# yeyupiaoling/MASR

Hardware: NVIDIA H100
Metric: audio_seconds_per_second (higher is better)
Workload: dtype f32 (GEMMs: fp16x2-split operands on wgmma, fp32 accumulate; fp32-grade results)

## Files before the change

include/masr_b200.h:

```cpp
#ifndef MASR_B200_H_
#define MASR_B200_H_

#include <stdint.h>

#ifdef __cplusplus
extern "C" {
#endif

#define MASR_ABI_VERSION 1

enum {
    MASR_OK = 0,
    MASR_ERR_INVALID_ARGUMENT = 10001,
    MASR_ERR_UNSUPPORTED_DEVICE = 10002,
    MASR_ERR_INTERNAL = 10003,
};

enum { MASR_STATUS_GAIN_EXCEEDED = 1 };

enum {
    MASR_EPI_BIAS = 0,
    MASR_EPI_BIAS_SILU = 1,
    MASR_EPI_BIAS_RELU = 2,
    MASR_EPI_BIAS_GLU = 3,
    MASR_EPI_BIAS_SCALE = 4,
    MASR_EPI_RESIDUAL = 5,
};

const char* masr_last_error(void);
int masr_abi_version(void);
int masr_check_device(void);


int masr_stage_waves_f32(const void* const* waves, const int64_t* lengths, int B, float* pinned, float* dev, int nthreads,
                         void* stream);

int masr_resample_f32(const float* x, const int64_t* x_offsets, const int* src_rates, int dst_rate, int B,
                      const double* table, int table_len, float* y, const int64_t* y_offsets, int64_t max_out,
                      int max_src_rate, void* stream);

int masr_fbank_workspace_bytes(int B, int64_t max_samples, int64_t* bytes_host);

int masr_wave_gain_f32(const float* wave, const int64_t* offsets, int B, int64_t max_samples, float target_db,
                       float max_gain_db, float* gain, int* status, void* workspace, void* stream);

int masr_fbank_f32(const float* wave, const int64_t* offsets, const float* gain, int B, int Fmax, float* feats,
                   int* num_frames, void* stream);


int masr_conv1_cmvn_relu_f32(const float* feats, const float* mean, const float* istd, const float* w1,
                             const float* b1, float* out, int B, int Fmax, int idim, int F1max, int W1, int C,
                             void* stream);

int masr_conv2_s2_relu_f32(const float* c1, const float* w2p, const float* b2, float* out, int B, int F1max,
                           int W1, int T2max, int W2, int C, void* stream);

int masr_gemm_f32(const float* A, int64_t lda, const float* W, const float* bias, const float* residual,
                  int64_t ldr, float* C, int64_t ldc, int M, int N, int K, int epilogue, float alpha,
                  void* stream);

int masr_gemm_tc_f16x2(const void* Ah, const void* Al, int64_t lda, const void* Wh, const void* Wl,
                       const float* bias, const float* residual, int64_t ldr, float* C, void* Ch, void* Cl,
                       int64_t ldc, int M, int N, int K, int epilogue, float alpha, void* stream);

int masr_ffn_tc_f16x2(const void* Ah, const void* Al, int64_t lda, const void* W1h, const void* W1l, const float* b1,
                      const void* W2h, const void* W2l, const float* b2, float* x, int64_t ldx, int M, int D, int F,
                      float alpha, void* stream);

int masr_gemm_tc_residual_ln_f16x2(const void* Ah, const void* Al, int64_t lda, const void* Wh, const void* Wl,
                                   const float* bias, const float* residual, int64_t ldr, float alpha, float* X,
                                   const float* gamma1, const float* beta1, const float* gamma2, const float* beta2,
                                   float* Y2, void* Yh, void* Yl, int64_t ldx, int M, int N, int K, float eps, void* stream);

int masr_gemm_tc_residual_postln_f16x2(const void* Ah, const void* Al, int64_t lda, const void* Wh, const void* Wl,
                                       const float* bias, const float* residual, int64_t ldr, float alpha, float* X,
                                       const float* gamma, const float* beta, const float* ada_scale, const float* ada_bias,
                                       void* Yh, void* Yl, int64_t ldx, int M, int N, int K, float eps, void* stream);

int masr_gemm_tc_lnpre_f16x2(const float* x, int64_t ldx, const float* gamma, const float* beta, float eps, void* Ah, void* Al,
                             int64_t lda, const void* Wh, const void* Wl, const float* bias, float* C, void* Ch, void* Cl,
                             int64_t ldc, int M, int N, int K, int epilogue, float alpha, void* stream);

int masr_ctc_head_argmax_tc_f16x2(const void* Ah, const void* Al, int64_t lda, const void* Wh, const void* Wl,
                                  const float* bias, int M, int V, int K, void* workspace, int64_t workspace_bytes,
                                  int* ids, float* maxp, void* stream);

int masr_conv1_cmvn_relu_planes_f16(const float* feats, const float* mean, const float* istd, const float* w1,
                                    const float* b1, void* planes_h, void* planes_l, int B, int Fmax, int idim,
                                    int F1max, int W1, int C, void* stream);
int masr_conv2_tc_f16x2(const void* c1h, const void* c1l, const void* Wh, const void* Wl, const float* bias,
                        float* out, void* outh, void* outl, int B, int F1, int T2, int C, void* stream);

int masr_split_f16(const float* x, void* h, void* l, int64_t n, void* stream);

int masr_layernorm_f32(const float* x, int64_t ldx, const float* gamma, const float* beta, float* y, int64_t ldy,
                       int M, int D, float eps, void* stream);

int masr_layernorm_split_f16(const float* x, int64_t ldx, const float* gamma, const float* beta, void* yh, void* yl,
                             int64_t ldy, int M, int D, float eps, void* stream);

int masr_layernorm2_split_f16(const float* x, int64_t ldx, const float* gamma1, const float* beta1, float* y1,
                              const float* gamma2, const float* beta2, float* y2, void* yh, void* yl, int64_t ldy, int M,
                              int D, float eps, void* stream);

int masr_layernorm_ada_split_f16(const float* x, int64_t ldx, const float* gamma, const float* beta, float* y,
                                 const float* ada_scale, const float* ada_bias, void* yh, void* yl, int64_t ldy, int M, int D,
                                 float eps, void* stream);
int masr_affine_split_f16(const float* x, const float* scale, const float* bias, void* yh, void* yl, int64_t M, int D,
                          void* stream);
int masr_dwconv_bn_silu_f32(const float* g, int64_t ldg, int64_t g_bstride, const float* w, const float* bias,
                            const float* bn_scale, const float* bn_shift, const float* pad_vec, float* y, void* yh, void* yl,
                            int64_t ldy, int64_t y_bstride, const int* in_lens, int B, int C, int kernel_size, int lpad,
                            int out_rows, void* stream);
int masr_time_reduce_dw_split_f16(const float* x, int64_t in_bstride, const float* w, const float* bias, void* yh, void* yl,
                                  int64_t out_bstride, const int* lens, int B, int out_rows, int k, int pad, int D,
                                  void* stream);
int masr_upsample2_add_f32(const float* saved, const float* z, float* out, int64_t full_bstride, int64_t half_bstride, int B,
                           int rows, int D, void* stream);

int masr_relpos_attention_f32(const float* Q, int64_t ldq, int64_t q_bstride, const float* K, const float* V,
                              int64_t ldk, int64_t k_bstride, const float* P, int64_t ldp, const float* pos_u,
                              const float* pos_v, float* O, void* Oh, void* Ol, int64_t ldo, int64_t o_bstride,
                              const int* q_lens, const int* k_lens, int B, int H, int d_k, int max_q, void* stream);

int masr_relpos_attention_tc(const float* Q, int64_t ldq, int64_t q_bstride, const void* Kh, const void* Kl, const void* Vh,
                             const void* Vl, int64_t ldk, int64_t k_bstride, const void* Ph, const void* Pl, int64_t ldp,
                             const float* pos_u, const float* pos_v, float* O, void* Oh, void* Ol, int64_t ldo,
                             int64_t o_bstride, const int* q_lens, const int* k_lens, int B, int H, int d_k, int max_q,
                             void* stream);

int masr_relpos_attention_tc5(const float* Q, int64_t ldq, int64_t q_bstride, const void* Kh, const void* Kl, const void* Vh,
                              const void* Vl, int64_t ldk, int64_t k_bstride, const void* Ph, const void* Pl, int64_t ldp,
                              int64_t table_rows, const float* pos_u, const float* pos_v, float* O, void* Oh, void* Ol,
                              int64_t ldo, int64_t o_bstride, const int* q_lens, const int* k_lens, int B, int H, int d_k,
                              int max_q, void* stream);

int masr_dwconv_ln_silu_f32(const float* g, int64_t ldg, int64_t g_bstride, const float* w, const float* bias,
                            const float* ln_gamma, const float* ln_beta, const float* pad_vec, float* y, void* yh,
                            void* yl, int64_t ldy, int64_t y_bstride, const int* in_lens, int B, int C,
                            int kernel_size, int lpad, int out_rows, float eps, void* stream);

int masr_dwconv_ln_silu_strided_f32(const float* g, int64_t ldg, int64_t g_bstride, const float* w, const float* bias,
                                    const float* ln_gamma, const float* ln_beta, const float* pad_vec, float* y, void* yh,
                                    void* yl, int64_t ldy, int64_t y_bstride, const int* in_lens, int B, int C,
                                    int kernel_size, int lpad, int stride, int out_rows, float eps, void* stream);

int masr_grouped_attention_f32(const float* Q, const float* K, const float* V, const float* P, int64_t ld, int64_t bstride,
                               const float* pos_u, const float* pos_v, float* O, void* Oh, void* Ol, const int* lens,
                               int B, int H, int d_k, int group, int max_t, void* stream);

int masr_grouped_attention_cache_f32(const float* Q, int64_t ldq, int64_t q_bstride, const float* K, const float* V,
                                     int64_t ldk, int64_t k_bstride, const float* P, const float* pos_u, const float* pos_v,
                                     float* O, void* Oh, void* Ol, const int* q_lens, const int* k_lens, int B, int H,
                                     int d_k, int group, int max_q, void* stream);

int masr_avgpool2_time_f32(const float* x, int64_t in_bstride, float* y, int64_t out_bstride, const int* lens, int B,
                           int out_rows, int D, void* stream);

int masr_lstm_step_f32(const float* gates_x, int64_t ldg, int64_t bstride, const float* Whh, const float* h_in_T,
                       float* h_out_T, float* c_state, float* out, void* outh, void* outl, int64_t ld_out, int col_off,
                       const int* lens, int B, int H, int step, int reverse, void* stream);

int masr_lstm_seq_workspace_bytes(int B, int H, int64_t* bytes);
int masr_lstm_seq_f32(const float* gates_x, int64_t ldg, int64_t bstride, const float* Whh, const float* h0_T, float* hN_T,
                      float* c_state, float* out, void* outh, void* outl, int64_t ld_out, int col_off, const int* lens, int B,
                      int H, int T, int reverse, void* workspace, int64_t workspace_bytes, void* stream);


int masr_stream_append_rows(const void* src0, const void* src1, int64_t src_pitch_bytes, int64_t col0_bytes, int row_bytes,
                            void* dst0, void* dst1, int64_t dst_pitch_bytes, int64_t cap, const int* base, const int* cnt,
                            int rows_per_slot, int S, void* stream);

int masr_stream_shift_cache(void* x0, void* x1, int64_t rows_per_slot, int lorder, int row_bytes, const int* cnt, int S,
                            void* stream);


int masr_ctc_frame_argmax_f32(const float* logits, int64_t ldl, int M, int V, int* ids, float* maxp, float* probs,
                              int64_t ldp, void* stream);

int masr_ctc_greedy_collapse(const int* ids, const float* maxp, int64_t bstride, const int* lens, int B, int blank,
                             int* tokens, int64_t tok_stride, int* ntok, float* psum, int* pcount, void* stream);

int masr_ctc_topk_f32(const float* logits, int64_t ldl, int M, int V, int top_n, float cutoff_prob, int* cand_id,
                      float* cand_logp, int* cand_cnt, void* stream);
int masr_ctc_prefix_beam_workspace(int B, int Tmax, int64_t* pool_floats_host, int64_t* trie_ints_per_utt_host);
int masr_ctc_prefix_beam(const int* cand_id, const float* cand_logp, const int* cand_cnt, int64_t bstride, const int* lens,
                         int B, int beam_size, int blank, float* pool, int* trie_parent, int* trie_tok, int64_t trie_cap,
                         int* out_tok, int64_t tok_stride, int* out_n, float* out_score, void* stream);

int masr_ctc_prefix_beam_state_size(int64_t* ints_per_utt, int64_t* floats_per_utt);
int masr_ctc_prefix_beam_stream(const int* cand_id, const float* cand_logp, const int* cand_cnt, int64_t bstride,
                                const int* lens, int B, int beam_size, int blank, float* pool, int* trie_parent,
                                int* trie_tok, int64_t trie_cap, int* state_i, float* state_f, int resume, int* out_tok,
                                int64_t tok_stride, int* out_n, float* out_score, void* stream);

typedef struct masr_lm_tables {
    const uint32_t* keys;
    const float* vals;
    const int* tok2lm;
    int order;
    int bos, eos;
    int vocab;
    int64_t off[8];
    int64_t mask[8];
} masr_lm_tables;

enum {
    MASR_LM_INFO_ORDER = 0, MASR_LM_INFO_CHAR_BASED = 1, MASR_LM_INFO_DICT_SIZE = 2, MASR_LM_INFO_VOCAB = 3,
    MASR_LM_INFO_KEY_WORDS = 4, MASR_LM_INFO_VAL_FLOATS = 5, MASR_LM_INFO_BOS = 6, MASR_LM_INFO_EOS = 7,
    MASR_LM_INFO_READ = 8,
    MASR_LM_INFO_KEPT = 14,
    MASR_LM_INFO_SLOTS = 20,
    MASR_LM_INFO_TABLE_BYTES = 26,
};

int masr_lm_load_arpa(const char* path_host, const char* vocab_host, int V, void** handle_host);
int masr_lm_info(const void* handle_host, int64_t* info_host);
int masr_lm_export(const void* handle_host, uint32_t* keys_host, float* vals_host, int* tok2lm_host,
                   masr_lm_tables* layout_host);
int masr_lm_free(void* handle_host);

int masr_lm_score_f32(const masr_lm_tables* lm_host, const int* ctx, const int* word, int Q, float* out, void* stream);

int masr_ctc_topk_blank_f32(const float* logits, int64_t ldl, int M, int V, int top_n, float cutoff_prob, int blank,
                            int* cand_id, float* cand_logp, int* cand_cnt, float* blank_logp, void* stream);

int masr_ctc_prefix_beam_lm(const int* cand_id, const float* cand_logp, const int* cand_cnt, const float* blank_logp,
                            int64_t bstride, const int* lens, int B, int beam_size, int blank, const masr_lm_tables* lm_host,
                            float alpha, float beta, float* pool, int* trie_parent, int* trie_tok, int64_t trie_cap,
                            int* out_tok, int64_t tok_stride, int* out_n, float* out_score, float* out_approx, void* stream);
int masr_ctc_prefix_beam_lm_state_size(int64_t* ints_per_utt, int64_t* floats_per_utt);
int masr_ctc_prefix_beam_lm_stream(const int* cand_id, const float* cand_logp, const int* cand_cnt, const float* blank_logp,
                                   int64_t bstride, const int* lens, int B, int beam_size, int blank,
                                   const masr_lm_tables* lm_host, float alpha, float beta, float* pool, int* trie_parent,
                                   int* trie_tok, int64_t trie_cap, int* state_i, float* state_f, int resume, int* out_tok,
                                   int64_t tok_stride, int* out_n, float* out_score, float* out_approx, void* stream);

int masr_ctc_prefix_beam_pool(const int* cand_id, const float* cand_logp, const int* cand_cnt, int64_t bstride,
                              const int* lens, int B, int beam_size, int blank, float* pool, int* trie_parent,
                              int* trie_tok, int64_t trie_cap, int* state_i, float* state_f, int* fresh, int* out_tok,
                              int64_t tok_stride, int* out_n, float* out_score, void* stream);
int masr_ctc_prefix_beam_lm_pool(const int* cand_id, const float* cand_logp, const int* cand_cnt, const float* blank_logp,
                                 int64_t bstride, const int* lens, int B, int beam_size, int blank,
                                 const masr_lm_tables* lm_host, float alpha, float beta, float* pool, int* trie_parent,
                                 int* trie_tok, int64_t trie_cap, int* state_i, float* state_f, int* fresh, int* out_tok,
                                 int64_t tok_stride, int* out_n, float* out_score, float* out_approx, void* stream);

#ifdef __cplusplus
}
#endif
#endif
```

masr_b200/_lib.py:

```python
from __future__ import annotations

import ctypes as C
import os
from typing import Optional

_HERE = os.path.dirname(os.path.abspath(__file__))
LIB_PATH = os.path.join(_HERE, "libmasr_b200.so")

OK = 0
EPI_BIAS, EPI_BIAS_SILU, EPI_BIAS_RELU, EPI_BIAS_GLU, EPI_BIAS_SCALE, EPI_RESIDUAL = range(6)
STATUS_GAIN_EXCEEDED = 1

_vp, _i, _i64, _f = C.c_void_p, C.c_int, C.c_int64, C.c_float


class LmTables(C.Structure):
    _fields_ = [("keys", _vp), ("vals", _vp), ("tok2lm", _vp), ("order", _i), ("bos", _i), ("eos", _i), ("vocab", _i),
                ("off", _i64 * 8), ("mask", _i64 * 8)]


_lmp = C.POINTER(LmTables)
LM_INFO_ORDER, LM_INFO_CHAR_BASED, LM_INFO_DICT_SIZE, LM_INFO_VOCAB, LM_INFO_KEY_WORDS, LM_INFO_VAL_FLOATS = range(6)
LM_INFO_READ, LM_INFO_KEPT, LM_INFO_SLOTS, LM_INFO_TABLE_BYTES = 8, 14, 20, 26

SIGNATURES = {
    "masr_abi_version": [],
    "masr_check_device": [],
    "masr_stage_waves_f32": [_vp, _vp, _i, _vp, _vp, _i, _vp],
    "masr_resample_f32": [_vp, _vp, _vp, _i, _i, _vp, _i, _vp, _vp, _i64, _i, _vp],
    "masr_fbank_workspace_bytes": [_i, _i64, C.POINTER(_i64)],
    "masr_wave_gain_f32": [_vp, _vp, _i, _i64, _f, _f, _vp, _vp, _vp, _vp],
    "masr_fbank_f32": [_vp, _vp, _vp, _i, _i, _vp, _vp, _vp],
    "masr_conv1_cmvn_relu_f32": [_vp, _vp, _vp, _vp, _vp, _vp, _i, _i, _i, _i, _i, _i, _vp],
    "masr_conv2_s2_relu_f32": [_vp, _vp, _vp, _vp, _i, _i, _i, _i, _i, _i, _vp],
    "masr_gemm_f32": [_vp, _i64, _vp, _vp, _vp, _i64, _vp, _i64, _i, _i, _i, _i, _f, _vp],
    "masr_gemm_tc_f16x2": [_vp, _vp, _i64, _vp, _vp, _vp, _vp, _i64, _vp, _vp, _vp, _i64, _i, _i, _i, _i, _f, _vp],
    "masr_ffn_tc_f16x2": [_vp, _vp, _i64, _vp, _vp, _vp, _vp, _vp, _vp, _vp, _i64, _i, _i, _i, _f, _vp],
    "masr_gemm_tc_residual_ln_f16x2": [_vp, _vp, _i64, _vp, _vp, _vp, _vp, _i64, _f, _vp, _vp, _vp, _vp, _vp, _vp, _vp, _vp, _i64,
                                       _i, _i, _i, _f, _vp],
    "masr_gemm_tc_residual_postln_f16x2": [_vp, _vp, _i64, _vp, _vp, _vp, _vp, _i64, _f, _vp, _vp, _vp, _vp, _vp, _vp, _vp, _i64,
                                           _i, _i, _i, _f, _vp],
    "masr_gemm_tc_lnpre_f16x2": [_vp, _i64, _vp, _vp, _f, _vp, _vp, _i64, _vp, _vp, _vp, _vp, _vp, _vp, _i64, _i, _i, _i, _i, _f,
                                 _vp],
    "masr_ctc_head_argmax_tc_f16x2": [_vp, _vp, _i64, _vp, _vp, _vp, _i, _i, _i, _vp, _i64, _vp, _vp, _vp],
    "masr_split_f16": [_vp, _vp, _vp, _i64, _vp],
    "masr_conv1_cmvn_relu_planes_f16": [_vp, _vp, _vp, _vp, _vp, _vp, _vp, _i, _i, _i, _i, _i, _i, _vp],
    "masr_conv2_tc_f16x2": [_vp, _vp, _vp, _vp, _vp, _vp, _vp, _vp, _i, _i, _i, _i, _vp],
    "masr_layernorm_f32": [_vp, _i64, _vp, _vp, _vp, _i64, _i, _i, _f, _vp],
    "masr_layernorm_split_f16": [_vp, _i64, _vp, _vp, _vp, _vp, _i64, _i, _i, _f, _vp],
    "masr_layernorm2_split_f16": [_vp, _i64, _vp, _vp, _vp, _vp, _vp, _vp, _vp, _vp, _i64, _i, _i, _f, _vp],
    "masr_layernorm_ada_split_f16": [_vp, _i64, _vp, _vp, _vp, _vp, _vp, _vp, _vp, _i64, _i, _i, _f, _vp],
    "masr_affine_split_f16": [_vp, _vp, _vp, _vp, _vp, _i64, _i, _vp],
    "masr_dwconv_bn_silu_f32": [_vp, _i64, _i64, _vp, _vp, _vp, _vp, _vp, _vp, _vp, _vp, _i64, _i64, _vp, _i, _i, _i, _i, _i, _vp],
    "masr_time_reduce_dw_split_f16": [_vp, _i64, _vp, _vp, _vp, _vp, _i64, _vp, _i, _i, _i, _i, _i, _vp],
    "masr_upsample2_add_f32": [_vp, _vp, _vp, _i64, _i64, _i, _i, _i, _vp],
    "masr_relpos_attention_f32": [_vp, _i64, _i64, _vp, _vp, _i64, _i64, _vp, _i64, _vp, _vp, _vp, _vp, _vp, _i64, _i64,
                                  _vp, _vp, _i, _i, _i, _i, _vp],
    "masr_relpos_attention_tc": [_vp, _i64, _i64, _vp, _vp, _vp, _vp, _i64, _i64, _vp, _vp, _i64, _vp, _vp, _vp, _vp, _vp, _i64,
                                 _i64, _vp, _vp, _i, _i, _i, _i, _vp],
    "masr_relpos_attention_tc5": [_vp, _i64, _i64, _vp, _vp, _vp, _vp, _i64, _i64, _vp, _vp, _i64, _i64, _vp, _vp, _vp, _vp, _vp,
                                  _i64, _i64, _vp, _vp, _i, _i, _i, _i, _vp],
    "masr_dwconv_ln_silu_f32": [_vp, _i64, _i64, _vp, _vp, _vp, _vp, _vp, _vp, _vp, _vp, _i64, _i64, _vp, _i, _i, _i, _i,
                                _i, _f, _vp],
    "masr_dwconv_ln_silu_strided_f32": [_vp, _i64, _i64, _vp, _vp, _vp, _vp, _vp, _vp, _vp, _vp, _i64, _i64, _vp, _i, _i, _i,
                                        _i, _i, _i, _f, _vp],
    "masr_grouped_attention_f32": [_vp, _vp, _vp, _vp, _i64, _i64, _vp, _vp, _vp, _vp, _vp, _vp, _i, _i, _i, _i, _i, _vp],
    "masr_grouped_attention_cache_f32": [_vp, _i64, _i64, _vp, _vp, _i64, _i64, _vp, _vp, _vp, _vp, _vp, _vp, _vp, _vp, _i, _i, _i,
                                         _i, _i, _vp],
    "masr_avgpool2_time_f32": [_vp, _i64, _vp, _i64, _vp, _i, _i, _i, _vp],
    "masr_lstm_step_f32": [_vp, _i64, _i64, _vp, _vp, _vp, _vp, _vp, _vp, _vp, _i64, _i, _vp, _i, _i, _i, _i, _vp],
    "masr_lstm_seq_workspace_bytes": [_i, _i, C.POINTER(_i64)],
    "masr_lstm_seq_f32": [_vp, _i64, _i64, _vp, _vp, _vp, _vp, _vp, _vp, _vp, _i64, _i, _vp, _i, _i, _i, _i, _vp, _i64, _vp],
    "masr_stream_append_rows": [_vp, _vp, _i64, _i64, _i, _vp, _vp, _i64, _i64, _vp, _vp, _i, _i, _vp],
    "masr_stream_shift_cache": [_vp, _vp, _i64, _i, _i, _vp, _i, _vp],
    "masr_ctc_frame_argmax_f32": [_vp, _i64, _i, _i, _vp, _vp, _vp, _i64, _vp],
    "masr_ctc_topk_f32": [_vp, _i64, _i, _i, _i, _f, _vp, _vp, _vp, _vp],
    "masr_ctc_prefix_beam_workspace": [_i, _i, C.POINTER(_i64), C.POINTER(_i64)],
    "masr_ctc_prefix_beam": [_vp, _vp, _vp, _i64, _vp, _i, _i, _i, _vp, _vp, _vp, _i64, _vp, _i64, _vp, _vp, _vp],
    "masr_ctc_prefix_beam_state_size": [C.POINTER(_i64), C.POINTER(_i64)],
    "masr_ctc_prefix_beam_stream": [_vp, _vp, _vp, _i64, _vp, _i, _i, _i, _vp, _vp, _vp, _i64, _vp, _vp, _i, _vp, _i64, _vp, _vp, _vp],
    "masr_ctc_greedy_collapse": [_vp, _vp, _i64, _vp, _i, _i, _vp, _i64, _vp, _vp, _vp, _vp],
    "masr_lm_load_arpa": [_vp, _vp, _i, C.POINTER(_vp)],
    "masr_lm_info": [_vp, C.POINTER(_i64)],
    "masr_lm_export": [_vp, _vp, _vp, _vp, _lmp],
    "masr_lm_free": [_vp],
    "masr_lm_score_f32": [_lmp, _vp, _vp, _i, _vp, _vp],
    "masr_ctc_topk_blank_f32": [_vp, _i64, _i, _i, _i, _f, _i, _vp, _vp, _vp, _vp, _vp],
    "masr_ctc_prefix_beam_lm": [_vp, _vp, _vp, _vp, _i64, _vp, _i, _i, _i, _lmp, _f, _f, _vp, _vp, _vp, _i64, _vp, _i64, _vp, _vp,
                                _vp, _vp],
    "masr_ctc_prefix_beam_lm_state_size": [C.POINTER(_i64), C.POINTER(_i64)],
    "masr_ctc_prefix_beam_lm_stream": [_vp, _vp, _vp, _vp, _i64, _vp, _i, _i, _i, _lmp, _f, _f, _vp, _vp, _vp, _i64, _vp, _vp, _i,
                                       _vp, _i64, _vp, _vp, _vp, _vp],
    "masr_ctc_prefix_beam_pool": [_vp, _vp, _vp, _i64, _vp, _i, _i, _i, _vp, _vp, _vp, _i64, _vp, _vp, _vp, _vp, _i64, _vp, _vp,
                                  _vp],
    "masr_ctc_prefix_beam_lm_pool": [_vp, _vp, _vp, _vp, _i64, _vp, _i, _i, _i, _lmp, _f, _f, _vp, _vp, _vp, _i64, _vp, _vp, _vp,
                                     _vp, _i64, _vp, _vp, _vp, _vp],
}


class MasrB200Error(RuntimeError):
    pass


_lib: Optional[C.CDLL] = None


def load() -> C.CDLL:
    global _lib
    if _lib is not None:
        return _lib
    if not os.path.exists(LIB_PATH):
        raise MasrB200Error(
            f"{LIB_PATH} not found: build it with `python -c 'import __graft_entry__ as g; g.build()'` "
            "(nvcc, sm_90a). masr_b200 has no CPU or PyTorch fallback.")
    lib = C.CDLL(LIB_PATH)
    lib.masr_last_error.restype = C.c_char_p
    lib.masr_last_error.argtypes = []
    for name, argtypes in SIGNATURES.items():
        fn = getattr(lib, name)
        fn.argtypes = argtypes
        fn.restype = C.c_int
    _lib = lib
    return lib


def last_error() -> str:
    return load().masr_last_error().decode("utf-8", "replace")


def check(rc: int, what: str):
    if rc != OK:
        raise MasrB200Error(f"{what} failed (code {rc}): {last_error()}")


def call(name: str, *args):
    check(getattr(load(), name)(*args), name)
```

masr_b200/csrc/ffn_tc.cu:

```cuda
#include <cuda.h>
#include <cuda_fp16.h>
#include <string.h>

#include "tc_common.cuh"

namespace masr {

namespace {

constexpr int FM = 64;
constexpr int FD = 256;
constexpr int FHC = 128;
constexpr int FBK = 32;
constexpr int F_STAGES = 4;
constexpr int F_STAGE_BYTES = 32768;
constexpr int F_H_BYTES = FM * FHC * 2 * 2;
constexpr int F_SUM_BYTES = FM * FD * 4;
constexpr int F_THREADS = 384;
constexpr int F_PRODUCER_REGS = 40, F_CONSUMER_REGS = 232;
constexpr uint32_t F_TX_A = 2 * FM * FBK * 2 + 2 * FHC * FBK * 2;
constexpr uint32_t F_TX_B = 2 * FD * FBK * 2;
constexpr size_t kFfnSmem = F_STAGES * F_STAGE_BYTES + F_H_BYTES + F_SUM_BYTES + 1024 + 256;
static_assert(kFfnSmem <= 232448, "ffn_tc shared memory exceeds the 227 KB per-CTA limit of sm_90");
static_assert(F_PRODUCER_REGS * 128 + F_CONSUMER_REGS * 256 <= 65536, "register file of the SM");

struct FfnMaps {
    CUtensorMap xh, xl;
    CUtensorMap w1h, w1l;
    CUtensorMap w2h, w2l;
};

struct FfnParams {
    const float* b1;
    const float* b2;
    float* x;
    int64_t ldx;
    int M, F;
    float alpha;
};

__device__ __forceinline__ void wgmma_m64n64k16_ss(float (&d)[32], uint64_t da, uint64_t db, uint32_t scale_d) {
    asm volatile(
        "{\n\t"
        ".reg .pred p;\n\t"
        "setp.ne.b32 p, %34, 0;\n\t"
        "wgmma.mma_async.sync.aligned.m64n64k16.f32.f16.f16 "
        "{%0, %1, %2, %3, %4, %5, %6, %7, %8, %9, %10, %11, %12, %13, %14, %15, "
        "%16, %17, %18, %19, %20, %21, %22, %23, %24, %25, %26, %27, %28, %29, %30, %31}, %32, %33, p, 1, 1, 0, 0;\n\t"
        "}"
        : "+f"(d[0]), "+f"(d[1]), "+f"(d[2]), "+f"(d[3]), "+f"(d[4]), "+f"(d[5]), "+f"(d[6]), "+f"(d[7]), "+f"(d[8]),
          "+f"(d[9]), "+f"(d[10]), "+f"(d[11]), "+f"(d[12]), "+f"(d[13]), "+f"(d[14]), "+f"(d[15]), "+f"(d[16]),
          "+f"(d[17]), "+f"(d[18]), "+f"(d[19]), "+f"(d[20]), "+f"(d[21]), "+f"(d[22]), "+f"(d[23]), "+f"(d[24]),
          "+f"(d[25]), "+f"(d[26]), "+f"(d[27]), "+f"(d[28]), "+f"(d[29]), "+f"(d[30]), "+f"(d[31])
        : "l"(da), "l"(db), "r"(scale_d));
}

__device__ __forceinline__ void bar_consumers() { asm volatile("bar.sync 1, 256;" ::: "memory"); }

__global__ void __launch_bounds__(F_THREADS, 1) ffn_tc_kernel(const __grid_constant__ FfnMaps maps, FfnParams p) {
    extern __shared__ uint8_t smem_raw[];
    uint8_t* smem = reinterpret_cast<uint8_t*>((reinterpret_cast<uintptr_t>(smem_raw) + 1023) & ~uintptr_t(1023));
    uint8_t* hbuf = smem + F_STAGES * F_STAGE_BYTES;
    uint8_t* sum = hbuf + F_H_BYTES;
    uint64_t* full_bar = reinterpret_cast<uint64_t*>(sum + F_SUM_BYTES);
    uint64_t* empty_bar = full_bar + F_STAGES;

    const int warp = threadIdx.x >> 5, lane = threadIdx.x & 31;
    const int nrb = (p.M + FM - 1) / FM;
    const int nch = p.F / FHC;

    if (warp == 8 && lane == 0) {
        tma_prefetch_desc(&maps.xh); tma_prefetch_desc(&maps.xl); tma_prefetch_desc(&maps.w1h);
        tma_prefetch_desc(&maps.w1l); tma_prefetch_desc(&maps.w2h); tma_prefetch_desc(&maps.w2l);
        for (int s = 0; s < F_STAGES; ++s) { mbar_init(&full_bar[s], 1); mbar_init(&empty_bar[s], 8); }
        asm volatile("fence.mbarrier_init.release.cluster;" ::: "memory");
    }
    __syncthreads();
    pdl_wait();
    pdl_launch_dependents();

    if (warp >= 8) {
        setmaxnreg_dec<F_PRODUCER_REGS>();
        if (warp == 8 && elect_one_sync()) {
            uint32_t kg = 0;
            auto acquire = [&](uint32_t tx) {
                const uint32_t s = kg % F_STAGES;
                mbar_wait(&empty_bar[s], ((kg / F_STAGES) & 1) ^ 1);
                mbar_expect_tx(&full_bar[s], tx);
                ++kg;
                return s;
            };
            for (int rb = blockIdx.x; rb < nrb; rb += gridDim.x) {
                const int m0 = rb * FM;
                for (int j = -1; j < nch; ++j) {
                    if (j >= 0) {
#pragma unroll 1
                        for (int kb = 0; kb < FHC / FBK; ++kb) {
                            const uint32_t s = acquire(F_TX_B);
                            uint8_t* st = smem + s * F_STAGE_BYTES;
                            tma_load_2d(&maps.w2h, &full_bar[s], st, j * FHC + kb * FBK, 0);
                            tma_load_2d(&maps.w2l, &full_bar[s], st + F_STAGE_BYTES / 2, j * FHC + kb * FBK, 0);
                        }
                    }
                    if (j + 1 < nch) {
#pragma unroll 1
                        for (int kb = 0; kb < FD / FBK; ++kb) {
                            const uint32_t s = acquire(F_TX_A);
                            uint8_t* st = smem + s * F_STAGE_BYTES;
                            tma_load_2d(&maps.xh, &full_bar[s], st, kb * FBK, m0);
                            tma_load_2d(&maps.xl, &full_bar[s], st + 4096, kb * FBK, m0);
                            tma_load_2d(&maps.w1h, &full_bar[s], st + 8192, kb * FBK, (j + 1) * FHC);
                            tma_load_2d(&maps.w1l, &full_bar[s], st + 16384, kb * FBK, (j + 1) * FHC);
                        }
                    }
                }
            }
        }
        __syncwarp();
    } else {
        setmaxnreg_inc<F_CONSUMER_REGS>();
        const int wg = warp >> 2, wi = warp & 3, q = lane & 3;
        const int tid = threadIdx.x & 127;
        const uint32_t h_base = smem_u32(hbuf);
        const uint32_t sum_base = smem_u32(sum) + wg * (F_SUM_BYTES / 2) + tid * 8;
        const uint32_t is_lane0 = lane == 0;
        auto release = [&](uint32_t s) {
            asm volatile("{\n\t.reg .pred p;\n\tsetp.ne.u32 p, %1, 0;\n\t@p mbarrier.arrive.shared::cta.b64 _, [%0];\n\t}"
                         ::"r"(smem_u32(&empty_bar[s])), "r"(is_lane0) : "memory");
        };
        float acc1[32], cor1[32], acc2[64], cor2[64];
        uint32_t kg = 0;
        int pend = -1;
        auto next_stage = [&]() {
            const uint32_t s = kg % F_STAGES;
            mbar_wait(&full_bar[s], (kg / F_STAGES) & 1);
            ++kg;
            return s;
        };
        auto retire = [&](uint32_t s) {
            wgmma_wait<1>();
            reg_fence(acc1); reg_fence(cor1); reg_fence(acc2); reg_fence(cor2);
            if (pend >= 0) release((uint32_t)pend);
            pend = (int)s;
        };
        auto phase_a = [&]() {
#pragma unroll 1
            for (int kb = 0; kb < FD / FBK; ++kb) {
                const uint32_t s = next_stage();
                const uint32_t sa = smem_u32(smem + s * F_STAGE_BYTES);
                const uint64_t dXh = gmma_desc_sw64(sa), dXl = gmma_desc_sw64(sa + 4096);
                const uint64_t dWh = gmma_desc_sw64(sa + 8192 + wg * 4096), dWl = gmma_desc_sw64(sa + 16384 + wg * 4096);
                reg_fence(acc1); reg_fence(cor1);
                wgmma_fence();
#pragma unroll
                for (int ks = 0; ks < FBK / 16; ++ks) {
                    const uint64_t adv = (uint64_t)(ks * 2);
                    const uint32_t first = (kb | ks) ? 1u : 0u;
                    wgmma_m64n64k16_ss(acc1, dXh + adv, dWh + adv, first);
                    wgmma_m64n64k16_ss(cor1, dXh + adv, dWl + adv, first);
                    wgmma_m64n64k16_ss(cor1, dXl + adv, dWh + adv, 1u);
                }
                wgmma_commit();
                retire(s);
            }
        };
        auto phase_b = [&](int j) {
#pragma unroll 1
            for (int kb = 0; kb < FHC / FBK; ++kb) {
                const uint32_t s = next_stage();
                const uint32_t sa = smem_u32(smem + s * F_STAGE_BYTES);
                const uint64_t dWh = gmma_desc_sw64(sa + wg * 8192), dWl = gmma_desc_sw64(sa + F_STAGE_BYTES / 2 + wg * 8192);
                const uint64_t dHh = gmma_desc_sw64(h_base + kb * 8192), dHl = gmma_desc_sw64(h_base + kb * 8192 + 4096);
                reg_fence(acc2); reg_fence(cor2);
                wgmma_fence();
#pragma unroll
                for (int ks = 0; ks < FBK / 16; ++ks) {
                    const uint64_t adv = (uint64_t)(ks * 2);
                    wgmma_m64n128k16_ss(acc2, dHh + adv, dWh + adv, ((j & 1) | kb | ks) ? 1u : 0u);
                    wgmma_m64n128k16_ss(cor2, dHh + adv, dWl + adv, (j | kb | ks) ? 1u : 0u);
                    wgmma_m64n128k16_ss(cor2, dHl + adv, dWh + adv, 1u);
                }
                wgmma_commit();
                retire(s);
            }
        };
        const int r_lo = 16 * wi + (lane >> 2);
        auto store_hidden = [&](int j) {
            float2 bb[8];
            const float* b = p.b1 + j * FHC + 64 * wg + 2 * q;
#pragma unroll
            for (int i = 0; i < 8; ++i) bb[i] = __ldg(reinterpret_cast<const float2*>(b + 8 * i));
#pragma unroll
            for (int i = 0; i < 8; ++i)
#pragma unroll
                for (int hh = 0; hh < 2; ++hh) {
                    float v0 = fmaf(cor1[4 * i + 2 * hh], kLoInv, acc1[4 * i + 2 * hh]);
                    float v1 = fmaf(cor1[4 * i + 2 * hh + 1], kLoInv, acc1[4 * i + 2 * hh + 1]);
                    v0 += bb[i].x; v1 += bb[i].y;
                    float e0, e1;
                    mul2(e0, e1, v0, v1, -1.4426950408889634f, -1.4426950408889634f);
                    e0 = ex2_approx(e0); e1 = ex2_approx(e1);
                    add2(e0, e1, e0, e1, 1.0f, 1.0f);
                    e0 = rcp_approx(e0); e1 = rcp_approx(e1);
                    mul2(v0, v1, v0, v1, e0, e1);
                    __half2 h2, l2;
                    split_f16x2(v0, v1, h2, l2);
                    const int r = r_lo + 8 * hh, c = 64 * wg + 8 * i + 2 * q;
                    const uint32_t a = h_base + (c >> 5) * 8192 + r * 64 + ((((c & 31) >> 3) ^ ((r >> 1) & 3)) << 4) + (c & 7) * 2;
                    asm volatile("st.shared.b32 [%0], %1;" ::"r"(a), "r"(*reinterpret_cast<uint32_t*>(&h2)) : "memory");
                    asm volatile("st.shared.b32 [%0], %1;" ::"r"(a + 4096), "r"(*reinterpret_cast<uint32_t*>(&l2)) : "memory");
                }
            asm volatile("fence.proxy.async.shared::cta;" ::: "memory");
        };
        auto drain = [&]() {
            wgmma_wait<0>();
            reg_fence(acc1); reg_fence(cor1); reg_fence(acc2); reg_fence(cor2);
            if (pend >= 0) release((uint32_t)pend);
            pend = -1;
        };

        for (int rb = blockIdx.x; rb < nrb; rb += gridDim.x) {
            const int m0 = rb * FM;
            phase_a();
            drain();
            bar_consumers();
            store_hidden(0);
            bar_consumers();
#pragma unroll 1
            for (int j = 0; j < nch; ++j) {
                phase_b(j);
                if (j + 1 < nch) phase_a();
                drain();
                if ((j & 1) && j + 1 < nch) {
#pragma unroll
                    for (int i = 0; i < 16; ++i)
#pragma unroll
                        for (int hh = 0; hh < 2; ++hh) {
                            float x0 = acc2[4 * i + 2 * hh], x1 = acc2[4 * i + 2 * hh + 1];
                            const uint32_t a = sum_base + (i * 2 + hh) * 1024;
                            if (j > 1) {
                                float s0, s1;
                                asm volatile("ld.shared.v2.f32 {%0, %1}, [%2];" : "=f"(s0), "=f"(s1) : "r"(a) : "memory");
                                x0 = s0 + x0; x1 = s1 + x1;
                            }
                            asm volatile("st.shared.v2.f32 [%0], {%1, %2};" ::"r"(a), "f"(x0), "f"(x1) : "memory");
                        }
                }
                if (j + 1 < nch) {
                    bar_consumers();
                    store_hidden(j + 1);
                    bar_consumers();
                }
            }
            const float* b2 = p.b2 + 128 * wg + 2 * q;
#pragma unroll
            for (int i = 0; i < 16; ++i) {
                const float2 bv = __ldg(reinterpret_cast<const float2*>(b2 + 8 * i));
#pragma unroll
                for (int hh = 0; hh < 2; ++hh) {
                    float x0 = acc2[4 * i + 2 * hh], x1 = acc2[4 * i + 2 * hh + 1];
                    if (nch > 2) {
                        float s0, s1;
                        asm volatile("ld.shared.v2.f32 {%0, %1}, [%2];" : "=f"(s0), "=f"(s1) : "r"(sum_base + (i * 2 + hh) * 1024) : "memory");
                        x0 = s0 + x0; x1 = s1 + x1;
                    }
                    x0 = fmaf(cor2[4 * i + 2 * hh], kLoInv, x0);
                    x1 = fmaf(cor2[4 * i + 2 * hh + 1], kLoInv, x1);
                    x0 += bv.x; x1 += bv.y;
                    const int row = m0 + r_lo + 8 * hh;
                    if (row < p.M) {
                        float2* xp = reinterpret_cast<float2*>(p.x + (int64_t)row * p.ldx + 128 * wg + 8 * i + 2 * q);
                        const float2 r = *xp;
                        x0 = r.x + p.alpha * x0;
                        x1 = r.y + p.alpha * x1;
                        *xp = make_float2(x0, x1);
                    }
                }
            }
        }
    }
    __syncthreads();
}

int ffn_map(CUtensorMap* map, const void* ptr, int64_t rows, int64_t K, int64_t ld, int box_rows) {
    EncodeTiledFn fn = get_encode_fn();
    if (!fn) { set_last_error("cuTensorMapEncodeTiled entry point unavailable"); return MASR_ERR_INTERNAL; }
    cuuint64_t dims[2] = {(cuuint64_t)K, (cuuint64_t)rows};
    cuuint64_t strides[1] = {(cuuint64_t)ld * 2};
    cuuint32_t box[2] = {(cuuint32_t)FBK, (cuuint32_t)box_rows};
    cuuint32_t estr[2] = {1, 1};
    CUresult r = fn(map, CU_TENSOR_MAP_DATA_TYPE_FLOAT16, 2, const_cast<void*>(ptr), dims, strides, box, estr,
                    CU_TENSOR_MAP_INTERLEAVE_NONE, CU_TENSOR_MAP_SWIZZLE_64B, CU_TENSOR_MAP_L2_PROMOTION_L2_128B,
                    CU_TENSOR_MAP_FLOAT_OOB_FILL_NONE);
    if (r != CUDA_SUCCESS) { set_last_error("cuTensorMapEncodeTiled failed (%d) rows=%lld K=%lld ld=%lld", (int)r, (long long)rows, (long long)K, (long long)ld); return MASR_ERR_INTERNAL; }
    return MASR_OK;
}

bool g_ffn_attr_set[64] = {false};

}

}

using namespace masr;

extern "C" int masr_ffn_tc_f16x2(const void* Ah, const void* Al, int64_t lda, const void* W1h, const void* W1l, const float* b1,
                                 const void* W2h, const void* W2l, const float* b2, float* x, int64_t ldx, int M, int D, int F,
                                 float alpha, void* stream) {
    if (M == 0) return MASR_OK;
    MASR_REQUIRE(Ah && Al && W1h && W1l && b1 && W2h && W2l && b2 && x, "masr_ffn_tc_f16x2: null pointer");
    MASR_REQUIRE(M > 0, "masr_ffn_tc_f16x2: M=%d", M);
    MASR_REQUIRE(D == FD, "masr_ffn_tc_f16x2: D=%d unsupported (this build: %d)", D, FD);
    MASR_REQUIRE(F > 0 && F % 256 == 0, "masr_ffn_tc_f16x2: F=%d must be a positive multiple of 256", F);
    MASR_REQUIRE(lda >= D && lda % 8 == 0, "masr_ffn_tc_f16x2: lda=%lld must be >= %d and a multiple of 8", (long long)lda, D);
    MASR_REQUIRE(ldx >= D && ldx % 2 == 0, "masr_ffn_tc_f16x2: ldx=%lld must be >= %d and even", (long long)ldx, D);
    MASR_REQUIRE(((reinterpret_cast<uintptr_t>(Ah) | reinterpret_cast<uintptr_t>(Al) | reinterpret_cast<uintptr_t>(W1h) |
                   reinterpret_cast<uintptr_t>(W1l) | reinterpret_cast<uintptr_t>(W2h) | reinterpret_cast<uintptr_t>(W2l)) & 15) == 0 &&
                 ((reinterpret_cast<uintptr_t>(x) | reinterpret_cast<uintptr_t>(b1) | reinterpret_cast<uintptr_t>(b2)) & 7) == 0,
                 "masr_ffn_tc_f16x2: misaligned pointer");
    FfnMaps maps;
    memset(&maps, 0, sizeof(maps));
    int rc;
    if ((rc = ffn_map(&maps.xh, Ah, M, D, lda, FM))) return rc;
    if ((rc = ffn_map(&maps.xl, Al, M, D, lda, FM))) return rc;
    if ((rc = ffn_map(&maps.w1h, W1h, F, D, D, FHC))) return rc;
    if ((rc = ffn_map(&maps.w1l, W1l, F, D, D, FHC))) return rc;
    if ((rc = ffn_map(&maps.w2h, W2h, D, F, F, FD))) return rc;
    if ((rc = ffn_map(&maps.w2l, W2l, D, F, F, FD))) return rc;
    int dev = 0;
    cudaGetDevice(&dev);
    if (dev < 0 || dev >= 64) dev = 0;
    if (!g_ffn_attr_set[dev]) {
        cudaError_t e = cudaFuncSetAttribute(ffn_tc_kernel, cudaFuncAttributeMaxDynamicSharedMemorySize, (int)kFfnSmem);
        if (e != cudaSuccess) { set_last_error("ffn_tc smem attr: %s", cudaGetErrorString(e)); return (int)e; }
        g_ffn_attr_set[dev] = true;
    }
    int sms = 0;
    if (cudaDeviceGetAttribute(&sms, cudaDevAttrMultiProcessorCount, dev) != cudaSuccess || sms <= 0) sms = 132;
    const int nrb = (M + FM - 1) / FM;
    FfnParams p{b1, b2, x, ldx, M, F, alpha};
    launch_pdl(ffn_tc_kernel, dim3(nrb < sms ? nrb : sms), dim3(F_THREADS), kFfnSmem, (cudaStream_t)stream, maps, p);
    return check_launch("ffn_tc_kernel");
}
```

masr_b200/csrc/tc_common.cuh:

```cuda
#pragma once
#include <cuda.h>
#include <cuda_fp16.h>
#include <mutex>

#include "common.cuh"

namespace masr {

constexpr float kLoScale = 2048.0f, kLoInv = 1.0f / 2048.0f;

__device__ __forceinline__ uint32_t smem_u32(const void* p) { return (uint32_t)__cvta_generic_to_shared(p); }

__device__ __forceinline__ void mbar_init(uint64_t* bar, uint32_t count) {
    asm volatile("mbarrier.init.shared::cta.b64 [%0], %1;" ::"r"(smem_u32(bar)), "r"(count));
}
__device__ __forceinline__ void mbar_expect_tx(uint64_t* bar, uint32_t bytes) {
    asm volatile("mbarrier.arrive.expect_tx.shared::cta.b64 _, [%0], %1;" ::"r"(smem_u32(bar)), "r"(bytes) : "memory");
}
__device__ __forceinline__ void mbar_wait(uint64_t* bar, uint32_t parity) {
    asm volatile(
        "{\n\t"
        ".reg .pred P1;\n\t"
        "WAIT_LOOP:\n\t"
        "mbarrier.try_wait.parity.shared::cta.b64 P1, [%0], %1;\n\t"
        "@P1 bra DONE;\n\t"
        "bra WAIT_LOOP;\n\t"
        "DONE:\n\t"
        "}" ::"r"(smem_u32(bar)), "r"(parity) : "memory");
}
__device__ __forceinline__ void tma_load_2d(const CUtensorMap* map, uint64_t* bar, void* smem_dst, int c0, int c1) {
    asm volatile(
        "cp.async.bulk.tensor.2d.shared::cluster.global.mbarrier::complete_tx::bytes [%0], [%1, {%3, %4}], [%2];"
        ::"r"(smem_u32(smem_dst)), "l"(map), "r"(smem_u32(bar)), "r"(c0), "r"(c1) : "memory");
}
__device__ __forceinline__ void tma_load_2d_mc(const CUtensorMap* map, uint64_t* bar, void* smem_dst, int c0, int c1, uint16_t mask) {
    asm volatile(
        "cp.async.bulk.tensor.2d.shared::cluster.global.mbarrier::complete_tx::bytes.multicast::cluster [%0], [%1, {%3, %4}], [%2], %5;"
        ::"r"(smem_u32(smem_dst)), "l"(map), "r"(smem_u32(bar)), "r"(c0), "r"(c1), "h"(mask) : "memory");
}
__device__ __forceinline__ void mbar_arrive_remote(uint64_t* bar, uint32_t rank) {
    uint32_t a;
    asm volatile("mapa.shared::cluster.u32 %0, %1, %2;" : "=r"(a) : "r"(smem_u32(bar)), "r"(rank));
    asm volatile("mbarrier.arrive.release.cluster.shared::cluster.b64 _, [%0];" ::"r"(a) : "memory");
}
__device__ __forceinline__ void tma_prefetch_desc(const CUtensorMap* map) {
    asm volatile("prefetch.tensormap [%0];" ::"l"(map) : "memory");
}
__device__ __forceinline__ bool elect_one_sync() {
    uint32_t pred = 0, laneid = 0;
    asm volatile(
        "{\n\t"
        ".reg .b32 %%rx;\n\t"
        ".reg .pred %%px;\n\t"
        "elect.sync %%rx|%%px, %2;\n\t"
        "@%%px mov.s32 %1, 1;\n\t"
        "mov.s32 %0, %%rx;\n\t"
        "}"
        : "+r"(laneid), "+r"(pred)
        : "r"(0xFFFFFFFFu));
    return pred != 0;
}

__device__ __forceinline__ void wgmma_fence() { asm volatile("wgmma.fence.sync.aligned;" ::: "memory"); }
__device__ __forceinline__ void wgmma_commit() { asm volatile("wgmma.commit_group.sync.aligned;" ::: "memory"); }
template <int N>
__device__ __forceinline__ void wgmma_wait() { asm volatile("wgmma.wait_group.sync.aligned %0;" ::"n"(N) : "memory"); }
template <int R>
__device__ __forceinline__ void reg_fence(float (&d)[R]) {
#pragma unroll
    for (int i = 0; i < R; ++i) asm volatile("" : "+f"(d[i])::"memory");
}
__device__ __forceinline__ void wgmma_m64n128k16_ss(float (&d)[64], uint64_t da, uint64_t db, uint32_t scale_d) {
    asm volatile(
        "{\n\t"
        ".reg .pred p;\n\t"
        "setp.ne.b32 p, %66, 0;\n\t"
        "wgmma.mma_async.sync.aligned.m64n128k16.f32.f16.f16 "
        "{%0, %1, %2, %3, %4, %5, %6, %7, %8, %9, %10, %11, %12, %13, %14, %15, "
        "%16, %17, %18, %19, %20, %21, %22, %23, %24, %25, %26, %27, %28, %29, %30, %31, "
        "%32, %33, %34, %35, %36, %37, %38, %39, %40, %41, %42, %43, %44, %45, %46, %47, "
        "%48, %49, %50, %51, %52, %53, %54, %55, %56, %57, %58, %59, %60, %61, %62, %63}, %64, %65, p, 1, 1, 0, 0;\n\t"
        "}"
        : "+f"(d[0]), "+f"(d[1]), "+f"(d[2]), "+f"(d[3]), "+f"(d[4]), "+f"(d[5]), "+f"(d[6]), "+f"(d[7]), "+f"(d[8]),
          "+f"(d[9]), "+f"(d[10]), "+f"(d[11]), "+f"(d[12]), "+f"(d[13]), "+f"(d[14]), "+f"(d[15]), "+f"(d[16]),
          "+f"(d[17]), "+f"(d[18]), "+f"(d[19]), "+f"(d[20]), "+f"(d[21]), "+f"(d[22]), "+f"(d[23]), "+f"(d[24]),
          "+f"(d[25]), "+f"(d[26]), "+f"(d[27]), "+f"(d[28]), "+f"(d[29]), "+f"(d[30]), "+f"(d[31]), "+f"(d[32]),
          "+f"(d[33]), "+f"(d[34]), "+f"(d[35]), "+f"(d[36]), "+f"(d[37]), "+f"(d[38]), "+f"(d[39]), "+f"(d[40]),
          "+f"(d[41]), "+f"(d[42]), "+f"(d[43]), "+f"(d[44]), "+f"(d[45]), "+f"(d[46]), "+f"(d[47]), "+f"(d[48]),
          "+f"(d[49]), "+f"(d[50]), "+f"(d[51]), "+f"(d[52]), "+f"(d[53]), "+f"(d[54]), "+f"(d[55]), "+f"(d[56]),
          "+f"(d[57]), "+f"(d[58]), "+f"(d[59]), "+f"(d[60]), "+f"(d[61]), "+f"(d[62]), "+f"(d[63])
        : "l"(da), "l"(db), "r"(scale_d));
}
template <int R>
__device__ __forceinline__ void setmaxnreg_inc() { asm volatile("setmaxnreg.inc.sync.aligned.u32 %0;" ::"n"(R)); }
template <int R>
__device__ __forceinline__ void setmaxnreg_dec() { asm volatile("setmaxnreg.dec.sync.aligned.u32 %0;" ::"n"(R)); }

__device__ __forceinline__ uint64_t gmma_desc_sw64(uint32_t smem_addr) {
    uint64_t d = 0;
    d |= (uint64_t)((smem_addr & 0x3FFFF) >> 4);
    d |= (uint64_t)1 << 16;
    d |= (uint64_t)(512 >> 4) << 32;
    d |= (uint64_t)2 << 62;
    return d;
}

__device__ __forceinline__ void add2(float& d0, float& d1, float a0, float a1, float b0, float b1) { d0 = a0 + b0; d1 = a1 + b1; }
__device__ __forceinline__ void sub2(float& d0, float& d1, float a0, float a1, float b0, float b1) { d0 = a0 - b0; d1 = a1 - b1; }
__device__ __forceinline__ void mul2(float& d0, float& d1, float a0, float a1, float b0, float b1) { d0 = a0 * b0; d1 = a1 * b1; }
__device__ __forceinline__ void split_f16(float x, __half& h, __half& l) {
    h = __float2half_rn(x);
    l = __float2half_rn((x - __half2float(h)) * kLoScale);
}
__device__ __forceinline__ void split_f16x2(float x0, float x1, __half2& h, __half2& l) {
    h = __floats2half2_rn(x0, x1);
    const float2 hf = __half22float2(h);
    float d0, d1;
    sub2(d0, d1, x0, x1, hf.x, hf.y);
    mul2(d0, d1, d0, d1, kLoScale, kLoScale);
    l = __floats2half2_rn(d0, d1);
}

__device__ __forceinline__ void mbar_arrive(uint64_t* bar) {
    asm volatile("mbarrier.arrive.shared::cta.b64 _, [%0];" ::"r"(smem_u32(bar)) : "memory");
}

__device__ __forceinline__ void sts128(uint32_t a, const uint4& v) {
    asm volatile("st.shared.v4.b32 [%0], {%1, %2, %3, %4};" ::"r"(a), "r"(v.x), "r"(v.y), "r"(v.z), "r"(v.w) : "memory");
}
__device__ __forceinline__ uint4 lds128(uint32_t a) {
    uint4 v;
    asm volatile("ld.shared.v4.b32 {%0, %1, %2, %3}, [%4];" : "=r"(v.x), "=r"(v.y), "=r"(v.z), "=r"(v.w) : "r"(a) : "memory");
    return v;
}

typedef CUresult (*EncodeTiledFn)(CUtensorMap*, CUtensorMapDataType, cuuint32_t, void*, const cuuint64_t*, const cuuint64_t*,
                                  const cuuint32_t*, const cuuint32_t*, CUtensorMapInterleave, CUtensorMapSwizzle,
                                  CUtensorMapL2promotion, CUtensorMapFloatOOBfill);

inline EncodeTiledFn get_encode_fn() {
    static EncodeTiledFn fn = nullptr;
    static std::once_flag once;
    std::call_once(once, [] {
        void* p = nullptr;
        cudaDriverEntryPointQueryResult qres;
        if (cudaGetDriverEntryPoint("cuTensorMapEncodeTiled", &p, cudaEnableDefault, &qres) == cudaSuccess &&
            qres == cudaDriverEntryPointSuccess)
            fn = reinterpret_cast<EncodeTiledFn>(p);
    });
    return fn;
}

}
```

masr_b200/csrc/tc_gemm.cu:

```cuda
#include <cuda.h>
#include <cuda_fp16.h>
#include <math.h>
#include <mutex>
#include <stdlib.h>
#include <string.h>

#include "tc_common.cuh"

namespace masr {

constexpr int TBM = 128, TBN = 128, TBK = 32;
constexpr int TILE_BYTES = TBM * TBK * 2;
constexpr int STAGE_BYTES = 4 * TILE_BYTES;
constexpr int EW = 8;
template <bool LNC> constexpr int kStages = LNC ? 4 : 5;
constexpr int RES_BYTES = TBM * TBN * 4;
constexpr int TC_THREADS = 32 * EW + 128;
constexpr int PRODUCER_REGS = 40, CONSUMER_REGS = 232;
static_assert(PRODUCER_REGS * 128 + CONSUMER_REGS * 32 * EW <= 65536, "register file of the SM");

struct TcParams {
    const float* bias;
    const float* residual;
    float* C;
    __half* Ch;
    __half* Cl;
    int64_t ldr, ldc;
    int M, N, K;
    int epi;
    float alpha;
    int conv_T2;
    int flags;
    const float* ln_g;
    const float* ln_b;
    const float* ln_g2;
    const float* ln_b2;
    float* y2;
    float ln_eps;
    float* part_m;
    float* part_s;
    int* part_i;
    const float* ada_s;
    const float* ada_b;
    const float* lnp_x;
    int64_t lnp_ldx, lnp_ld;
    __half* lnp_h;
    __half* lnp_l;
};

__device__ __forceinline__ void ln_row256_split(const float4 (&v)[2], const float* __restrict__ gamma, const float* __restrict__ beta,
                                                float eps, int lane, __half* __restrict__ yh, __half* __restrict__ yl) {
    float s = 0.f;
#pragma unroll
    for (int i = 0; i < 2; ++i) s += (v[i].x + v[i].y) + (v[i].z + v[i].w);
    const float mean = warp_sum(s) * (1.0f / 256);
    float q = 0.f;
#pragma unroll
    for (int i = 0; i < 2; ++i) {
        float a = v[i].x - mean, b = v[i].y - mean, c = v[i].z - mean, d = v[i].w - mean;
        q += (a * a + b * b) + (c * c + d * d);
    }
    const float rstd = rsqrtf(warp_sum(q) * (1.0f / 256) + eps);
#pragma unroll
    for (int i = 0; i < 2; ++i) {
        const int c = (i * 32 + lane) * 4;
        float4 g = ldg_f4(gamma + c), b = ldg_f4(beta + c);
        float4 o;
        o.x = (v[i].x - mean) * rstd * g.x + b.x;
        o.y = (v[i].y - mean) * rstd * g.y + b.y;
        o.z = (v[i].z - mean) * rstd * g.z + b.z;
        o.w = (v[i].w - mean) * rstd * g.w + b.w;
        __half hh[4], ll[4];
        const float ov[4] = {o.x, o.y, o.z, o.w};
#pragma unroll
        for (int j = 0; j < 4; ++j) {
            hh[j] = __float2half_rn(ov[j]);
            ll[j] = __float2half_rn((ov[j] - __half2float(hh[j])) * 2048.0f);
        }
        *reinterpret_cast<uint2*>(yh + c) = *reinterpret_cast<const uint2*>(hh);
        *reinterpret_cast<uint2*>(yl + c) = *reinterpret_cast<const uint2*>(ll);
    }
}

constexpr int EPI_RESIDUAL_LN = 6, EPI_RESIDUAL_LN2 = 7, EPI_CTC_PARTIAL = 8, EPI_RESIDUAL_POSTLN = 9;

struct TcMaps {
    CUtensorMap a[8];
    CUtensorMap w[2];
};

constexpr int CHUNK_KB = 256 / TBK;
constexpr int CONV_TR = 6, CONV_W2 = 19, CONV_ROWS = CONV_TR * CONV_W2;

__device__ __forceinline__ void tma_load_4d(const CUtensorMap* map, uint64_t* bar, void* smem_dst, int c0, int c1, int c2, int c3) {
    asm volatile(
        "cp.async.bulk.tensor.4d.shared::cluster.global.mbarrier::complete_tx::bytes [%0], [%1, {%3, %4, %5, %6}], [%2];"
        ::"r"(smem_u32(smem_dst)), "l"(map), "r"(smem_u32(bar)), "r"(c0), "r"(c1), "r"(c2), "r"(c3) : "memory");
}

struct EpiCtx {
    uint32_t sb;
    int lane;
    int64_t row0;
    int nvalid;
};

template <int CH>
__device__ __forceinline__ void staged_store(const EpiCtx& c, const uint4 (&regs)[CH], uint8_t* g0, int64_t pitch_bytes) {
    constexpr int RSH = (CH == 8) ? 0 : (CH == 4) ? 1 : 2;
    constexpr int RPI = 32 / CH;
    __syncwarp();
#pragma unroll
    for (int k = 0; k < CH; ++k) sts128(c.sb + c.lane * (CH * 16) + ((k ^ ((c.lane >> RSH) & (CH - 1))) << 4), regs[k]);
    __syncwarp();
    const int sub = c.lane / CH, k = c.lane % CH;
    uint4 v[CH];
#pragma unroll
    for (int i = 0; i < CH; ++i) {
        const int row = i * RPI + sub;
        v[i] = lds128(c.sb + row * (CH * 16) + ((k ^ ((row >> RSH) & (CH - 1))) << 4));
    }
#pragma unroll
    for (int i = 0; i < CH; ++i) {
        const int row = i * RPI + sub;
        if (row < c.nvalid) *reinterpret_cast<uint4*>(g0 + row * pitch_bytes + (k << 4)) = v[i];
    }
}

__device__ __forceinline__ void staged_load(const EpiCtx& c, uint4 (&regs)[8], const uint8_t* g0, int64_t pitch_bytes) {
    __syncwarp();
    const int sub = c.lane >> 3, k = c.lane & 7;
    uint4 v[8];
#pragma unroll
    for (int i = 0; i < 8; ++i) {
        const int row = i * 4 + sub;
        v[i] = make_uint4(0, 0, 0, 0);
        if (row < c.nvalid) v[i] = *reinterpret_cast<const uint4*>(g0 + row * pitch_bytes + (k << 4));
    }
#pragma unroll
    for (int i = 0; i < 8; ++i) {
        const int row = i * 4 + sub;
        sts128(c.sb + row * 128 + ((k ^ (row & 7)) << 4), v[i]);
    }
    __syncwarp();
#pragma unroll
    for (int k2 = 0; k2 < 8; ++k2) regs[k2] = lds128(c.sb + c.lane * 128 + ((k2 ^ (c.lane & 7)) << 4));
}

template <int W, int STG>
__device__ __forceinline__ void emit_f32(const EpiCtx& c, float* C, int64_t ld, int flags, const float (&o)[W], int n, int n_limit) {
    const bool full = n + W - 1 < n_limit;
    const bool row_ok = c.lane < c.nvalid;
    const int64_t my_row = c.row0 + c.lane;
    if ((flags & 1) && full && (ld & 3) == 0 && (reinterpret_cast<uintptr_t>(C) & 15) == 0) {
        constexpr int CH = (W / 4 < STG / 512) ? W / 4 : STG / 512;
#pragma unroll
        for (int part = 0; part < (W / 4) / CH; ++part) {
            uint4 regs[CH];
#pragma unroll
            for (int j = 0; j < CH; ++j) {
                const int e = (part * CH + j) * 4;
                regs[j] = make_uint4(__float_as_uint(o[e]), __float_as_uint(o[e + 1]), __float_as_uint(o[e + 2]), __float_as_uint(o[e + 3]));
            }
            staged_store<CH>(c, regs, reinterpret_cast<uint8_t*>(C + c.row0 * ld + n + part * CH * 4), ld * 4);
        }
    } else if (row_ok && full && (ld & 3) == 0 && (reinterpret_cast<uintptr_t>(C) & 15) == 0) {
        float* cp = C + my_row * ld + n;
#pragma unroll
        for (int j = 0; j < W; j += 4) *reinterpret_cast<float4*>(cp + j) = make_float4(o[j], o[j + 1], o[j + 2], o[j + 3]);
    } else if (row_ok) {
        float* cp = C + my_row * ld + n;
#pragma unroll
        for (int j = 0; j < W; ++j)
            if (n + j < n_limit) cp[j] = o[j];
    }
}

template <int W, int STG>
__device__ __forceinline__ void emit_pair(const EpiCtx& c, __half* Ch, __half* Cl, int64_t ld, int flags, const float (&o)[W], int n,
                                          int n_limit) {
    const bool full = n + W - 1 < n_limit;
    const bool row_ok = c.lane < c.nvalid;
    const int64_t my_row = c.row0 + c.lane;
    uint32_t hh[W / 2], ll[W / 2];
#pragma unroll
    for (int j = 0; j < W / 2; ++j) {
        __half2 h2, l2;
        split_f16x2(o[2 * j], o[2 * j + 1], h2, l2);
        hh[j] = *reinterpret_cast<uint32_t*>(&h2);
        ll[j] = *reinterpret_cast<uint32_t*>(&l2);
    }
    const bool aligned = (ld & 7) == 0 && ((reinterpret_cast<uintptr_t>(Ch) | reinterpret_cast<uintptr_t>(Cl)) & 15) == 0;
    if ((flags & 1) && full && aligned) {
        constexpr int CH = (W / 8 < STG / 512) ? W / 8 : STG / 512;
#pragma unroll
        for (int part = 0; part < (W / 8) / CH; ++part) {
            uint4 regs[CH];
#pragma unroll
            for (int j = 0; j < CH; ++j) { const int e = 4 * (part * CH + j); regs[j] = make_uint4(hh[e], hh[e + 1], hh[e + 2], hh[e + 3]); }
            staged_store<CH>(c, regs, reinterpret_cast<uint8_t*>(Ch + c.row0 * ld + n + part * CH * 8), ld * 2);
#pragma unroll
            for (int j = 0; j < CH; ++j) { const int e = 4 * (part * CH + j); regs[j] = make_uint4(ll[e], ll[e + 1], ll[e + 2], ll[e + 3]); }
            staged_store<CH>(c, regs, reinterpret_cast<uint8_t*>(Cl + c.row0 * ld + n + part * CH * 8), ld * 2);
        }
    } else if (row_ok && full && aligned) {
        uint4* hp = reinterpret_cast<uint4*>(Ch + my_row * ld + n);
        uint4* lp = reinterpret_cast<uint4*>(Cl + my_row * ld + n);
#pragma unroll
        for (int j = 0; j < W / 8; ++j) {
            hp[j] = make_uint4(hh[4 * j], hh[4 * j + 1], hh[4 * j + 2], hh[4 * j + 3]);
            lp[j] = make_uint4(ll[4 * j], ll[4 * j + 1], ll[4 * j + 2], ll[4 * j + 3]);
        }
    } else if (row_ok) {
        unsigned short* hp = reinterpret_cast<unsigned short*>(Ch + my_row * ld + n);
        unsigned short* lp = reinterpret_cast<unsigned short*>(Cl + my_row * ld + n);
#pragma unroll
        for (int j = 0; j < W / 2; ++j) {
            if (n + 2 * j < n_limit) { hp[2 * j] = (unsigned short)(hh[j] & 0xffff); lp[2 * j] = (unsigned short)(ll[j] & 0xffff); }
            if (n + 2 * j + 1 < n_limit) { hp[2 * j + 1] = (unsigned short)(hh[j] >> 16); lp[2 * j + 1] = (unsigned short)(ll[j] >> 16); }
        }
    }
}

template <int W, int STG>
__device__ __forceinline__ void emit(const TcParams& p, const EpiCtx& c, const float (&o)[W], int n, int n_limit) {
    if (p.C) emit_f32<W, STG>(c, p.C, p.ldc, p.flags, o, n, n_limit);
    if (p.Ch) emit_pair<W, STG>(c, p.Ch, p.Cl, p.ldc, p.flags, o, n, n_limit);
}

struct LnCtx {
    uint32_t red, red_peer;
    uint32_t bar, bar_peer;
    uint32_t rank, cgrp, row, lane;
    uint32_t round;
};

__device__ __forceinline__ void ln_apply(LnCtx& L, const float (&v)[32], float (&o)[32], const float* g, const float* b, float eps) {
    float s = 0.f;
#pragma unroll
    for (int j = 0; j < 32; j += 4) s += (v[j] + v[j + 1]) + (v[j + 2] + v[j + 3]);
    const float m_loc = s * (1.0f / 32.0f);
    float q = 0.f;
#pragma unroll
    for (int j = 0; j < 32; j += 4) {
        const float a0 = v[j] - m_loc, a1 = v[j + 1] - m_loc, a2 = v[j + 2] - m_loc, a3 = v[j + 3] - m_loc;
        q += (a0 * a0 + a1 * a1) + (a2 * a2 + a3 * a3);
    }
    const uint32_t buf = L.round & 1;
    const uint32_t off = ((((buf * 2 + L.rank) * 4 + L.cgrp) * 128) + L.row) * 8;
    asm volatile("st.shared.v2.f32 [%0], {%1, %2};" ::"r"(L.red + off), "f"(m_loc), "f"(q) : "memory");
    asm volatile("st.shared::cluster.v2.f32 [%0], {%1, %2};" ::"r"(L.red_peer + off), "f"(m_loc), "f"(q) : "memory");
    __syncwarp();
    if (L.lane == 0) {
        asm volatile("mbarrier.arrive.release.cluster.shared::cluster.b64 _, [%0];" ::"r"(L.bar + buf * 8) : "memory");
        asm volatile("mbarrier.arrive.release.cluster.shared::cluster.b64 _, [%0];" ::"r"(L.bar_peer + buf * 8) : "memory");
    }
    const uint32_t parity = (L.round >> 1) & 1;
    asm volatile(
        "{\n\t"
        ".reg .pred P1;\n\t"
        "LN_WAIT:\n\t"
        "mbarrier.try_wait.parity.acquire.cluster.shared::cta.b64 P1, [%0], %1;\n\t"
        "@P1 bra LN_DONE;\n\t"
        "bra LN_WAIT;\n\t"
        "LN_DONE:\n\t"
        "}" ::"r"(L.bar + buf * 8), "r"(parity) : "memory");
    float pm[8], pq[8];
#pragma unroll
    for (int k = 0; k < 8; ++k)
        asm volatile("ld.shared.v2.f32 {%0, %1}, [%2];" : "=f"(pm[k]), "=f"(pq[k]) : "r"(L.red + (((buf * 8 + k) * 128) + L.row) * 8) : "memory");
    ++L.round;
    const float mean = (((pm[0] + pm[1]) + (pm[2] + pm[3])) + ((pm[4] + pm[5]) + (pm[6] + pm[7]))) * 0.125f;
    float m2 = ((pq[0] + pq[1]) + (pq[2] + pq[3])) + ((pq[4] + pq[5]) + (pq[6] + pq[7]));
    float dev2 = 0.f;
#pragma unroll
    for (int k = 0; k < 8; ++k) { const float dm = pm[k] - mean; dev2 += dm * dm; }
    m2 = fmaf(32.0f, dev2, m2);
    const float rstd = rsqrtf(m2 * (1.0f / 256.0f) + eps);
#pragma unroll
    for (int j = 0; j < 32; j += 4) {
        const float4 gg = ldg_f4(g + j), bb = ldg_f4(b + j);
        o[j] = (v[j] - mean) * rstd * gg.x + bb.x;
        o[j + 1] = (v[j + 1] - mean) * rstd * gg.y + bb.y;
        o[j + 2] = (v[j + 2] - mean) * rstd * gg.z + bb.z;
        o[j + 3] = (v[j + 3] - mean) * rstd * gg.w + bb.w;
    }
}

template <int STG, bool LNC>
__device__ __forceinline__ void store_chunk(const TcParams& p, const EpiCtx& c, float (&v)[32], int n, LnCtx& L) {
    constexpr bool BIG = STG >= 4096;
    if (!LNC && p.epi == EPI_CTC_PARTIAL) {
        if (n + 31 >= p.N) {
#pragma unroll
            for (int j = 0; j < 32; ++j)
                if (n + j >= p.N) v[j] = -INFINITY;
        }
        float m = v[0];
#pragma unroll
        for (int j = 1; j < 32; ++j) m = fmaxf(m, v[j]);
        int mj = 31;
#pragma unroll
        for (int j = 30; j >= 0; --j)
            if (v[j] == m) mj = j;
        const int mi = n + mj;
        const float mneg = -m * 1.4426950408889634f;
        float sum = 0.f;
#pragma unroll
        for (int j = 0; j < 32; ++j) sum += ex2_approx(fmaf(v[j], 1.4426950408889634f, mneg));
        if (c.lane < c.nvalid) {
            const int64_t idx = (int64_t)(n >> 5) * p.M + c.row0 + c.lane;
            p.part_m[idx] = m; p.part_s[idx] = sum; p.part_i[idx] = mi;
        }
        return;
    }
    if (p.epi == MASR_EPI_BIAS_GLU) {
        float o[16];
#pragma unroll
        for (int j = 0; j < 16; j += 8) {
            float e[8];
#pragma unroll
            for (int k = 0; k < 8; ++k) e[k] = ex2_approx(v[2 * (j + k) + 1] * -1.4426950408889634f);
#pragma unroll
            for (int k = 0; k < 8; ++k) e[k] = rcp_approx(1.0f + e[k]);
#pragma unroll
            for (int k = 0; k < 8; ++k) o[j + k] = v[2 * (j + k)] * e[k];
        }
        emit<16, STG>(p, c, o, n >> 1, p.N >> 1);
        return;
    }
    switch (LNC ? (int)MASR_EPI_RESIDUAL : p.epi) {
        case MASR_EPI_BIAS_SILU:
#pragma unroll
            for (int j = 0; j < 32; j += 8) {
                float e[8];
#pragma unroll
                for (int k = 0; k < 8; k += 2) mul2(e[k], e[k + 1], v[j + k], v[j + k + 1], -1.4426950408889634f, -1.4426950408889634f);
#pragma unroll
                for (int k = 0; k < 8; ++k) e[k] = ex2_approx(e[k]);
#pragma unroll
                for (int k = 0; k < 8; k += 2) add2(e[k], e[k + 1], e[k], e[k + 1], 1.0f, 1.0f);
#pragma unroll
                for (int k = 0; k < 8; ++k) e[k] = rcp_approx(e[k]);
#pragma unroll
                for (int k = 0; k < 8; k += 2) mul2(v[j + k], v[j + k + 1], v[j + k], v[j + k + 1], e[k], e[k + 1]);
            }
            break;
        case MASR_EPI_BIAS_RELU:
#pragma unroll
            for (int j = 0; j < 32; ++j) v[j] = fmaxf(v[j], 0.f);
            break;
        case MASR_EPI_BIAS_SCALE:
#pragma unroll
            for (int j = 0; j < 32; ++j) v[j] *= p.alpha;
            break;
        case MASR_EPI_RESIDUAL: {
            const bool vec_r = (p.ldr & 3) == 0 && (reinterpret_cast<uintptr_t>(p.residual) & 15) == 0;
            if (BIG && (p.flags & 2) && n + 31 < p.N && vec_r) {
                uint4 rr[8];
                staged_load(c, rr, reinterpret_cast<const uint8_t*>(p.residual + c.row0 * p.ldr + n), p.ldr * 4);
#pragma unroll
                for (int j = 0; j < 8; ++j) {
                    v[4 * j] = __uint_as_float(rr[j].x) + p.alpha * v[4 * j];
                    v[4 * j + 1] = __uint_as_float(rr[j].y) + p.alpha * v[4 * j + 1];
                    v[4 * j + 2] = __uint_as_float(rr[j].z) + p.alpha * v[4 * j + 2];
                    v[4 * j + 3] = __uint_as_float(rr[j].w) + p.alpha * v[4 * j + 3];
                }
            } else if (c.lane < c.nvalid && n + 31 < p.N && vec_r) {
                const float* r = p.residual + (c.row0 + c.lane) * p.ldr + n;
#pragma unroll
                for (int j = 0; j < 32; j += 4) {
                    const float4 rv = *reinterpret_cast<const float4*>(r + j);
                    v[j] = rv.x + p.alpha * v[j]; v[j + 1] = rv.y + p.alpha * v[j + 1];
                    v[j + 2] = rv.z + p.alpha * v[j + 2]; v[j + 3] = rv.w + p.alpha * v[j + 3];
                }
            } else if (c.lane < c.nvalid) {
                const float* r = p.residual + (c.row0 + c.lane) * p.ldr + n;
#pragma unroll
                for (int j = 0; j < 32; ++j)
                    if (n + j < p.N) v[j] = r[j] + p.alpha * v[j];
            }
            break;
        }
        default: break;
// ... 653 lines not shown
```

masr_b200/engine.py:

```python
from __future__ import annotations

import os
from dataclasses import dataclass
from typing import Dict, List, Optional, Sequence, Tuple

import numpy as np
import torch

from . import _lib
from . import resample as resampling
from ._lib import EPI_BIAS, EPI_BIAS_GLU, EPI_BIAS_SCALE, EPI_BIAS_SILU, EPI_RESIDUAL, call
from .weights import ConformerWeights, load_state_dict, pack_conformer

FRAME_LEN, FRAME_SHIFT, NUM_MEL = 400, 160, 80
_NVTX = os.environ.get("MASR_NVTX", "0") == "1"


def num_frames(num_samples: int) -> int:
    return 0 if num_samples < FRAME_LEN else 1 + (num_samples - FRAME_LEN) // FRAME_SHIFT


def subsampled_len(frames: int) -> int:
    return max(0, ((frames - 1) // 2 - 1) // 2)


def check_max_len(out_lens: Sequence[int], max_len: int) -> None:
    m = max(out_lens) if len(out_lens) else 0
    if max_len > 0 and m >= max_len:
        raise AssertionError("offset: {} + x.shape[1]: {} is larger than the max_len: {}".format(0, m, max_len))


def _p(t: Optional[torch.Tensor]):
    return None if t is None else t.data_ptr()


@dataclass
class GreedyResult:
    tokens: List[List[int]]
    scores: List[float]
    frame_ids: Optional[np.ndarray] = None
    frame_lens: Optional[np.ndarray] = None
    status: Optional[np.ndarray] = None


class ConformerEngine:

    def __init__(self, weights_src, streaming: bool = True, device: str = "cuda", max_len: int = 5000,
                 gemm: str = "tc", use_graphs: bool = True):
        if gemm not in ("tc", "simt"):
            raise ValueError("gemm must be 'tc' or 'simt'")
        self.gemm_path = gemm
        self.fuse_ctc = os.environ.get("MASR_FUSE_CTC", "1") != "0"
        self.attn_tc5 = os.environ.get("MASR_ATTN", "tc5") != "mma"
        self.fuse = os.environ.get("MASR_FUSE_LN", "0") == "1"
        self.lnpre = os.environ.get("MASR_FUSE_LNPRE", "0") == "1"
        self.use_graphs = bool(use_graphs)
        self._graphs = {}
        if not torch.cuda.is_available():
            raise _lib.MasrB200Error("masr_b200 needs a CUDA device (sm_90a); there is no CPU fallback")
        self.lib = _lib.load()
        dev = torch.device(device)
        if dev.index is None:
            dev = torch.device("cuda", torch.cuda.current_device())
        self.device = dev
        torch.cuda.set_device(self.device)
        call("masr_check_device")
        sd = load_state_dict(weights_src)
        self.w: ConformerWeights = self._pack(sd, max_len)
        self.causal = bool(streaming)
        self.d, self.h = self.w.d_model, self.w.heads
        self.dk = self.d // self.h
        self.V = self.w.vocab
        self.Vpad = (self.V + 15) // 16 * 16
        self.f2 = ((self.w.idim - 1) // 2 - 1) // 2
        self.w1_cols = (self.w.idim - 1) // 2
        self._ws: Dict[Tuple, Dict[str, torch.Tensor]] = {}
        self.launches = 0
        self._pinned: Optional[torch.Tensor] = None
        self._out_pinned: Optional[torch.Tensor] = None
        self._staged: Optional[torch.cuda.Event] = None
        self._rs_in: Dict[str, torch.Tensor] = {}
        self.h2d_bytes = 0
        self.d2h_bytes = 0
        self.last_gain = None
        self.prof: Optional[Dict[str, list]] = None
        self.graph_tail_hook = None
        self._precompute_pos()
        self._tcw = {}
        if self.gemm_path == "tc":
            self._split_weights()

    def _pack(self, sd, max_len):
        return pack_conformer(sd, self.device, max_len)

    def _split(self, x: torch.Tensor):
        x = x.contiguous()
        h = torch.empty(x.shape, dtype=torch.float16, device=self.device)
        l = torch.empty(x.shape, dtype=torch.float16, device=self.device)
        call("masr_split_f16", _p(x), _p(h), _p(l), x.numel(), self._stream())
        return h, l

    def _split_weights(self):
        w = self.w
        t = self._tcw
        t["conv2"] = self._split(w.conv2_w)
        t["embed"] = self._split(w.embed_w)
        t["ctc"] = self._split(w.ctc_w)
        for i, L in enumerate(w.layers):
            t[i, "ffm1"] = self._split(L.ffm[0]); t[i, "ffm2"] = self._split(L.ffm[2])
            t[i, "qkv"] = self._split(L.wqkv); t[i, "wo"] = self._split(L.wo)
            t[i, "pw1"] = self._split(L.pw1); t[i, "pw2"] = self._split(L.pw2)
            t[i, "ff1"] = self._split(L.ff[0]); t[i, "ff2"] = self._split(L.ff[2])
        torch.cuda.synchronize(self.device)

    def _ptab_pair(self, L):
        if getattr(L, "ptab_p", None) is None or L.ptab_p[2] is not L.ptab:
            h, l = self._split(L.ptab)
            L.ptab_p = (h, l, L.ptab)
        return L.ptab_p

    def _attention_tc(self, L, qkv, qkvp, outp, T, lens, B):
        d = self.d
        ph, pl, _ = self._ptab_pair(L)
        if T <= 256 and self.dk == 64 and self.attn_tc5:
            self._k("attention", "masr_relpos_attention_tc5", _p(qkv), 3 * d, T, qkvp[0].data_ptr() + 2 * d, qkvp[1].data_ptr() + 2 * d,
                    qkvp[0].data_ptr() + 4 * d, qkvp[1].data_ptr() + 4 * d, 3 * d, T, _p(ph), _p(pl), d, ph.shape[0], _p(L.pos_u),
                    _p(L.pos_v), None, _p(outp[0]), _p(outp[1]), d, T, _p(lens), _p(lens), B, self.h, self.dk, T)
            return
        self._k("attention", "masr_relpos_attention_tc", _p(qkv), 3 * d, T, qkvp[0].data_ptr() + 2 * d, qkvp[1].data_ptr() + 2 * d,
                qkvp[0].data_ptr() + 4 * d, qkvp[1].data_ptr() + 4 * d, 3 * d, T, _p(ph), _p(pl), d, _p(L.pos_u), _p(L.pos_v), None,
                _p(outp[0]), _p(outp[1]), d, T, _p(lens), _p(lens), B, self.h, self.dk, T)

    def _tc(self, A, lda, W, bias, M, N, K, epi=EPI_BIAS, alpha=1.0, residual=None, ldr=0, C=None, Cp=None, ldc=0,
            tag="gemm"):
        self._k(tag, "masr_gemm_tc_f16x2", _p(A[0]), _p(A[1]), lda, _p(W[0]), _p(W[1]), _p(bias), _p(residual), ldr,
                _p(C), None if Cp is None else _p(Cp[0]), None if Cp is None else _p(Cp[1]), ldc, M, N, K, epi, alpha)

    def _tc_ln(self, A, lda, W, bias, M, K, alpha, x, ln1, yp, ln2=None, y2=None, tag="gemm"):
        d = self.d
        self._k(tag, "masr_gemm_tc_residual_ln_f16x2", _p(A[0]), _p(A[1]), lda, _p(W[0]), _p(W[1]), _p(bias), _p(x), d, alpha,
                _p(x), _p(ln1[0]), _p(ln1[1]), None if ln2 is None else _p(ln2[0]), None if ln2 is None else _p(ln2[1]),
                _p(y2), _p(yp[0]), _p(yp[1]), d, M, d, K, 1e-5)

    def _tc_postln(self, A, lda, W, bias, M, K, x, ln, ada, yp, alpha=1.0, tag="gemm"):
        d = self.d
        self._k(tag, "masr_gemm_tc_residual_postln_f16x2", _p(A[0]), _p(A[1]), lda, _p(W[0]), _p(W[1]), _p(bias), _p(x), d, alpha,
                _p(x), _p(ln[0]), _p(ln[1]), None if ada is None else _p(ada[0]), None if ada is None else _p(ada[1]),
                _p(yp[0]), _p(yp[1]), d, M, d, K, 1e-5)

    def _ffn_fused(self) -> bool:
        return self.gemm_path == "tc" and not self.fuse and self.d == 256 and self.w.ffn % 256 == 0

    def _ffn_tc(self, A, W1, b1, W2, b2, M, x, alpha=0.5):
        d = self.d
        self._k("ffn_fused", "masr_ffn_tc_f16x2", _p(A[0]), _p(A[1]), d, _p(W1[0]), _p(W1[1]), _p(b1), _p(W2[0]), _p(W2[1]),
                _p(b2), _p(x), d, M, d, self.w.ffn, alpha)

    def _hidp(self, ws):
        if "hidp" not in ws:
            Mx, f16 = ws["x"].shape[0], torch.float16
            ws["hidp"] = (torch.empty(Mx, self.w.ffn, device=self.device, dtype=f16),
                          torch.empty(Mx, self.w.ffn, device=self.device, dtype=f16))
        return ws["hidp"]

    def time_ffn_gemms(self, ws, M: int, reps: int = 12, iters: int = 5) -> float:
        w, d, tw, L = self.w, self.d, self._tcw, self.w.layers[0]
        t0p = ws["t0p"]
        xs = torch.zeros_like(ws["x"])
        dev = self.device
        fused = self._ffn_fused()

        def body():
            for _ in range(reps):
                if fused:
                    self._ffn_tc(t0p, tw[0, "ffm1"], L.ffm[1], tw[0, "ffm2"], L.ffm[3], M, xs)
                    continue
                hidp = self._hidp(ws)
                self._tc(t0p, d, tw[0, "ffm1"], L.ffm[1], M, w.ffn, d, EPI_BIAS_SILU, Cp=hidp, ldc=w.ffn, tag="ffn_w1")
                self._tc(hidp, w.ffn, tw[0, "ffm2"], L.ffm[3], M, d, w.ffn, EPI_RESIDUAL, 0.5, xs, d, C=xs, ldc=d, tag="ffn_w2")

        prof, self.prof = self.prof, None
        n0 = self.launches
        side = torch.cuda.Stream(device=dev)
        side.wait_stream(torch.cuda.current_stream(dev))
        with torch.cuda.stream(side):
            body()
        torch.cuda.current_stream(dev).wait_stream(side)
        torch.cuda.synchronize(dev)
        g = torch.cuda.CUDAGraph()
        with torch.cuda.graph(g, capture_error_mode="thread_local"):
            body()
        best = float("inf")
        for _ in range(iters):
            xs.zero_()
            e0, e1 = torch.cuda.Event(enable_timing=True), torch.cuda.Event(enable_timing=True)
            e0.record()
            g.replay()
            e1.record()
            e1.synchronize()
            best = min(best, e0.elapsed_time(e1))
        self.launches, self.prof = n0, prof
        return best / (2 * reps)

    def _ln_tc(self, x, gb, yp, W, bias, M, N, epi=EPI_BIAS, C=None, Cp=None, ldc=0, tag="gemm"):
        d = self.d
        if self.lnpre and d == 256:
            self._k(tag, "masr_gemm_tc_lnpre_f16x2", _p(x), d, _p(gb[0]), _p(gb[1]), 1e-5, _p(yp[0]), _p(yp[1]), d, _p(W[0]),
                    _p(W[1]), _p(bias), _p(C), None if Cp is None else _p(Cp[0]), None if Cp is None else _p(Cp[1]), ldc, M, N, d,
                    epi, 1.0)
            return
        self._ln_split(x, gb, yp, M)
        self._tc(yp, d, W, bias, M, N, d, epi, C=C, Cp=Cp, ldc=ldc, tag=tag)

    def _ln_split(self, x, gb, yp, M):
        self._k("layernorm", "masr_layernorm_split_f16", _p(x), self.d, _p(gb[0]), _p(gb[1]), _p(yp[0]), _p(yp[1]),
                self.d, M, self.d, 1e-5)

    def _stream(self):
        return torch.cuda.current_stream(self.device).cuda_stream

    def _gemm(self, A, lda, W, bias, C, ldc, M, N, K, epi=EPI_BIAS, alpha=1.0, residual=None, ldr=0, tag="gemm"):
        ev = self._prof_begin(tag)
        call("masr_gemm_f32", _p(A), lda, _p(W), _p(bias), _p(residual), ldr, _p(C), ldc, M, N, K, epi, alpha,
             self._stream())
        self._prof_end(ev)
        self.launches += 1

    def _k(self, tag, name, *args, n=1):
        ev = self._prof_begin(tag)
        if _NVTX:
            torch.cuda.nvtx.range_push(tag)
        call(name, *args, self._stream())
        if _NVTX:
            torch.cuda.nvtx.range_pop()
        self._prof_end(ev)
        self.launches += n

    def _prof_begin(self, tag):
        if self.prof is None:
            return None
        e0 = torch.cuda.Event(enable_timing=True)
        e1 = torch.cuda.Event(enable_timing=True)
        e0.record(torch.cuda.current_stream(self.device))
        self.prof.setdefault(tag, []).append((e0, e1))
        return e1

    def _prof_end(self, ev):
        if ev is not None:
            ev.record(torch.cuda.current_stream(self.device))

    def profile(self, enable: bool):
        self.prof = {} if enable else None

    def profile_summary(self) -> Dict[str, Tuple[int, float]]:
        out = {}
        for tag, evs in (self.prof or {}).items():
            out[tag] = (len(evs), float(sum(a.elapsed_time(b) for a, b in evs)))
        fused = out.pop("ffn_fused", None)
        if fused is not None:
            for tag in ("ffn_w1", "ffn_w2"):
                n, ms = out.get(tag, (0, 0.0))
                out[tag] = (n + fused[0], ms + 0.5 * fused[1])
        return out

    def _ln(self, x, gb, y, M, ld=None):
        ld = self.d if ld is None else ld
        self._k("layernorm", "masr_layernorm_f32", _p(x), ld, _p(gb[0]), _p(gb[1]), _p(y), ld, M, self.d, 1e-5)

    def _precompute_pos(self):
        for L in self.w.layers:
            L.ptab = torch.empty(self.w.max_len, self.d, device=self.device, dtype=torch.float32)
            self._gemm(self.w.pe, self.d, L.wpos, None, L.ptab, self.d, self.w.max_len, self.d, self.d)
        torch.cuda.synchronize(self.device)

    def _workspace(self, B: int, Fmax: int) -> Dict[str, torch.Tensor]:
        key = (B, Fmax)
        ws = self._ws.get(key)
        if ws is not None:
            return ws
        dev, f32 = self.device, torch.float32
        F1 = (Fmax - 1) // 2
        T = subsampled_len(Fmax)
        M = B * T
        d = self.d
        ws = {
            "c1": torch.empty(B * F1 * self.w1_cols * d, device=dev, dtype=f32),
            "c2": torch.empty(max(1, M) * self.f2 * d, device=dev, dtype=f32),
            "x": torch.empty(max(1, M), d, device=dev, dtype=f32),
            "t0": torch.empty(max(1, M), d, device=dev, dtype=f32),
            "t1": torch.empty(max(1, M), d, device=dev, dtype=f32),
            "g": torch.empty(max(1, M), d, device=dev, dtype=f32),
            "hid": torch.empty(max(1, M), self.w.ffn, device=dev, dtype=f32),
            "qkv": torch.empty(max(1, M), 3 * d, device=dev, dtype=f32),
            "logits": torch.empty(max(1, M), self.Vpad, device=dev, dtype=f32),
            "ids": torch.empty(max(1, M), device=dev, dtype=torch.int32),
            "maxp": torch.empty(max(1, M), device=dev, dtype=f32),
        }
        self._alloc_out_pack(ws, B, T)
        if self.gemm_path == "tc":
            f16 = torch.float16
            TH = (F1 + 1) // 2
            Mx = max(1, M)
            del ws["c1"], ws["c2"], ws["hid"]
            ws["c1p"] = (torch.zeros(4 * B * TH * 20 * d, device=dev, dtype=f16), torch.zeros(4 * B * TH * 20 * d, device=dev, dtype=f16))
            ws["c2p"] = (torch.empty(Mx * self.f2, d, device=dev, dtype=f16), torch.empty(Mx * self.f2, d, device=dev, dtype=f16))
            ws["t0p"] = (torch.empty(Mx, d, device=dev, dtype=f16), torch.empty(Mx, d, device=dev, dtype=f16))
            ws["t1p"] = (torch.empty(Mx, d, device=dev, dtype=f16), torch.empty(Mx, d, device=dev, dtype=f16))
            ws["qkvp"] = (torch.empty(Mx, 3 * d, device=dev, dtype=f16), torch.empty(Mx, 3 * d, device=dev, dtype=f16))
        if len(self._ws) > 8:
            self._ws.clear()
        self._ws[key] = ws
        return ws

    def _alloc_out_pack(self, ws, B: int, T: int):
        Tt = max(1, T)
        pack = torch.zeros(B * Tt + 4 * B, device=self.device, dtype=torch.int32)
        ws["out_pack"] = pack
        ws["tokens"] = pack[:B * Tt].view(B, Tt)
        ws["ntok"] = pack[B * Tt:B * Tt + B]
        ws["pcount"] = pack[B * Tt + B:B * Tt + 2 * B]
        ws["status"] = pack[B * Tt + 2 * B:B * Tt + 3 * B]
        ws["psum"] = pack[B * Tt + 3 * B:].view(torch.float32)

    def fbank(self, waves: Sequence[np.ndarray], use_db_normalization: bool = True, target_db: float = -20.0,
              wave_dev: Optional[torch.Tensor] = None, offsets_dev: Optional[torch.Tensor] = None,
              lengths: Optional[Sequence[int]] = None, force_fmax: Optional[int] = None,
              status_out: Optional[torch.Tensor] = None, rates: Optional[Sequence[int]] = None):
        if wave_dev is None:
            lengths = [int(w.shape[0]) for w in waves]
            nb = len(waves)
            offs = np.zeros(nb + 1, np.int64)
            np.cumsum(lengths, out=offs[1:])
            total = int(offs[-1])
            tail_f = 2 * (nb + 1)
            if self._staged is not None:
                self._staged.synchronize()
            if self._pinned is None or self._pinned.numel() < total + tail_f + 2:
                n = (int(1.25 * total) + tail_f + 1024) // 2 * 2
                self._pinned = torch.empty(n, dtype=torch.float32, pin_memory=True)
            hv = self._pinned.numpy()
            for i, w in enumerate(waves):
                hv[offs[i]:offs[i + 1]] = w
            t0 = (total + 1) // 2 * 2
            self._pinned[t0:t0 + tail_f].view(torch.int64).copy_(torch.from_numpy(offs))
            wave_dev = self._pinned[:max(1, total)].to(self.device, non_blocking=True)
            offsets_dev = self._pinned[t0:t0 + tail_f].view(torch.int64).to(self.device, non_blocking=True)
            self._staged = torch.cuda.Event()
            self._staged.record(torch.cuda.current_stream(self.device))
            self.h2d_bytes += 4 * total + 8 * (nb + 1)
            if resampling.needs_resampling(rates):
                wave_dev, offsets_dev, lengths = self._resample_packed(wave_dev, offsets_dev, lengths, rates)
        B = len(lengths)
        frames = [num_frames(n) for n in lengths]
        Fmax = max(frames) if frames else 0
        if force_fmax is not None:
            Fmax = int(force_fmax)
        max_samples = max(lengths) if lengths else 0
        dev = self.device
        feats = torch.empty(B, max(1, Fmax), NUM_MEL, device=dev, dtype=torch.float32)
        if status_out is not None:
            status = status_out
            status.zero_()
        else:
            status = torch.zeros(B, device=dev, dtype=torch.int32)
        gain = None
        self.last_gain = None
        if use_db_normalization:
            nbytes = _lib.C.c_int64(0)
            call("masr_fbank_workspace_bytes", B, max_samples, _lib.C.byref(nbytes))
            scratch = torch.empty(max(8, nbytes.value), device=dev, dtype=torch.uint8)
            gain = torch.empty(B, device=dev, dtype=torch.float32)
            self._k("wave_gain", "masr_wave_gain_f32", _p(wave_dev), _p(offsets_dev), B, max_samples, float(target_db),
                    300.0, _p(gain), _p(status), _p(scratch), n=2)
            self.last_gain = gain
        if Fmax > 0:
            self._k("fbank", "masr_fbank_f32", _p(wave_dev), _p(offsets_dev), _p(gain), B, Fmax, _p(feats), None)
        return feats, frames, status

    def _resample_packed(self, x, x_offs, lengths, rates):
        rates = [int(r) for r in rates]
        out_lengths = [resampling.output_length(n, r) for n, r in zip(lengths, rates)]
        offs = resampling.offsets(out_lengths)
        y = torch.empty(max(1, int(offs[-1])), device=self.device, dtype=torch.float32)
        y_offs = torch.from_numpy(offs).to(self.device)
        rates_dev = torch.tensor(rates, dtype=torch.int32).to(self.device)
        self.h2d_bytes += 8 * len(offs) + 4 * len(rates)
        resampling.launch(self, x, x_offs, rates_dev, y, y_offs, rates, out_lengths)
        return y, y_offs, out_lengths

    def resample(self, waves: Sequence[np.ndarray], rates: Sequence[int]) -> List[np.ndarray]:
        lengths = [int(w.shape[0]) for w in waves]
        if not waves:
            return []
        x = torch.from_numpy(np.concatenate([np.asarray(w, np.float32) for w in waves]) if sum(lengths) else
                             np.zeros(1, np.float32)).to(self.device)
        x_offs = torch.from_numpy(resampling.offsets(lengths)).to(self.device)
        self.h2d_bytes += 4 * sum(lengths) + 8 * (len(lengths) + 1)
        y, _, out_lengths = self._resample_packed(x, x_offs, lengths, rates)
        yh = y.cpu().numpy()
        self.d2h_bytes += 4 * sum(out_lengths)
        offs = resampling.offsets(out_lengths)
        return [yh[offs[i]:offs[i + 1]].copy() for i in range(len(waves))]

    def encode(self, feats: torch.Tensor, feat_lens: Sequence[int], tlens_dev: Optional[torch.Tensor] = None):
        w = self.w
        B, Fmax = feats.shape[0], feats.shape[1]
        F1 = (Fmax - 1) // 2
        T = subsampled_len(Fmax)
        tl = [subsampled_len(int(f)) for f in feat_lens]
        if tlens_dev is None:
            check_max_len(tl, self.w.max_len)
        ws = self._workspace(B, Fmax)
        if T == 0:
            return ws["x"][:0], tl, 0, ws
        M, d = B * T, self.d
        if tlens_dev is not None:
            ws["tlens"] = tlens_dev
            ws["tl_host"] = None
        elif ws.get("tl_host") != tl:
            ws["tlens"] = torch.tensor(tl, dtype=torch.int32, device=self.device)
            ws["tl_host"] = list(tl)
            self.h2d_bytes += 4 * B
        tlens = ws["tlens"]
        if self.gemm_path == "tc":
            return self._encode_tc(feats, ws, tl, tlens, B, Fmax, F1, T, M)
        self._k("conv1", "masr_conv1_cmvn_relu_f32", _p(feats), _p(w.cmvn_mean), _p(w.cmvn_istd), _p(w.conv1_w),
                _p(w.conv1_b), _p(ws["c1"]), B, Fmax, w.idim, F1, self.w1_cols, d)
        self._k("conv2", "masr_conv2_s2_relu_f32", _p(ws["c1"]), _p(w.conv2_w), _p(w.conv2_b), _p(ws["c2"]), B, F1,
                self.w1_cols, T, self.f2, d)
        x, t0, t1, g, hid, qkv = ws["x"], ws["t0"], ws["t1"], ws["g"], ws["hid"], ws["qkv"]
        self._gemm(ws["c2"], self.f2 * d, w.embed_w, w.embed_b, x, d, M, d, self.f2 * d, EPI_BIAS_SCALE, float(d) ** 0.5,
                   tag="embed_linear")
        lpad = (w.kernel - 1) if self.causal else (w.kernel - 1) // 2
        for L in w.layers:
            self._ln(x, L.ln_ffm, t0, M)
            self._gemm(t0, d, L.ffm[0], L.ffm[1], hid, w.ffn, M, w.ffn, d, EPI_BIAS_SILU, tag="ffn_w1")
            self._gemm(hid, w.ffn, L.ffm[2], L.ffm[3], x, d, M, d, w.ffn, EPI_RESIDUAL, 0.5, x, d, tag="ffn_w2")
            self._ln(x, L.ln_mha, t0, M)
            self._gemm(t0, d, L.wqkv, L.bqkv, qkv, 3 * d, M, 3 * d, d, tag="qkv_proj")
            self._k("attention", "masr_relpos_attention_f32", _p(qkv), 3 * d, T, qkv.data_ptr() + 4 * d,
                    qkv.data_ptr() + 8 * d, 3 * d, T, _p(L.ptab), d, _p(L.pos_u), _p(L.pos_v), _p(t1), None, None, d, T,
                    _p(tlens), _p(tlens), B, self.h, self.dk, T)
            self._gemm(t1, d, L.wo, L.bo, x, d, M, d, d, EPI_RESIDUAL, 1.0, x, d, tag="out_proj")
            self._ln(x, L.ln_conv, t0, M)
            self._gemm(t0, d, L.pw1, L.pw1_b, g, d, M, 2 * d, d, EPI_BIAS_GLU, tag="pw1_glu")
            self._k("dwconv_ln_silu", "masr_dwconv_ln_silu_f32", _p(g), d, T, _p(L.dw), _p(L.dw_b), _p(L.cn[0]),
                    _p(L.cn[1]), _p(L.glu_pad) if self.causal else None, _p(t1), None, None, d, T, _p(tlens), B, d,
                    w.kernel, lpad, T, 1e-5)
            self._gemm(t1, d, L.pw2, L.pw2_b, x, d, M, d, d, EPI_RESIDUAL, 1.0, x, d, tag="pw2")
            self._ln(x, L.ln_ff, t0, M)
            self._gemm(t0, d, L.ff[0], L.ff[1], hid, w.ffn, M, w.ffn, d, EPI_BIAS_SILU, tag="ffn_w1")
            self._gemm(hid, w.ffn, L.ff[2], L.ff[3], x, d, M, d, w.ffn, EPI_RESIDUAL, 0.5, x, d, tag="ffn_w2")
            self._ln(x, L.ln_final, x, M)
        self._ln(x, w.after_norm, t0, M)
        return t0[:M], tl, T, ws

    def _encode_tc(self, feats, ws, tl, tlens, B, Fmax, F1, T, M):
        w, d, tw = self.w, self.d, self._tcw
        x, g, qkv = ws["x"], ws["g"], ws["qkv"]
        t0p, t1p, c1p, c2p = ws["t0p"], ws["t1p"], ws["c1p"], ws["c2p"]
        ffn_fused = self._ffn_fused()
        hidp = None if ffn_fused else self._hidp(ws)
        self._k("conv1", "masr_conv1_cmvn_relu_planes_f16", _p(feats), _p(w.cmvn_mean), _p(w.cmvn_istd), _p(w.conv1_w),
                _p(w.conv1_b), _p(c1p[0]), _p(c1p[1]), B, Fmax, w.idim, F1, self.w1_cols, d)
        self._k("conv2", "masr_conv2_tc_f16x2", _p(c1p[0]), _p(c1p[1]), _p(tw["conv2"][0]), _p(tw["conv2"][1]),
                _p(w.conv2_b), None, _p(c2p[0]), _p(c2p[1]), B, F1, T, d)
        self._tc(c2p, self.f2 * d, tw["embed"], w.embed_b, M, d, self.f2 * d, EPI_BIAS_SCALE, float(d) ** 0.5, C=x, ldc=d,
                 tag="embed_linear")
        lpad = (w.kernel - 1) if self.causal else (w.kernel - 1) // 2
        nl = len(w.layers)
        for i, L in enumerate(w.layers):
            fuse = self.fuse and d == 256
            if ffn_fused:
                if i == 0:
                    self._ln_split(x, L.ln_ffm, t0p, M)
                self._ffn_tc(t0p, tw[i, "ffm1"], L.ffm[1], tw[i, "ffm2"], L.ffm[3], M, x)
            elif i == 0:
                self._ln_tc(x, L.ln_ffm, t0p, tw[i, "ffm1"], L.ffm[1], M, w.ffn, EPI_BIAS_SILU, Cp=hidp, ldc=w.ffn, tag="ffn_w1")
            else:
                self._tc(t0p, d, tw[i, "ffm1"], L.ffm[1], M, w.ffn, d, EPI_BIAS_SILU, Cp=hidp, ldc=w.ffn, tag="ffn_w1")
            if fuse:
                self._tc_ln(hidp, w.ffn, tw[i, "ffm2"], L.ffm[3], M, w.ffn, 0.5, x, L.ln_mha, t0p, tag="ffn_w2")
            elif not ffn_fused:
                self._tc(hidp, w.ffn, tw[i, "ffm2"], L.ffm[3], M, d, w.ffn, EPI_RESIDUAL, 0.5, x, d, C=x, ldc=d, tag="ffn_w2")
            if fuse:
                self._tc(t0p, d, tw[i, "qkv"], L.bqkv, M, 3 * d, d, C=qkv, Cp=ws["qkvp"], ldc=3 * d, tag="qkv_proj")
            else:
                self._ln_tc(x, L.ln_mha, t0p, tw[i, "qkv"], L.bqkv, M, 3 * d, C=qkv, Cp=ws["qkvp"], ldc=3 * d, tag="qkv_proj")
            self._attention_tc(L, qkv, ws["qkvp"], t1p, T, tlens, B)
            if fuse:
                self._tc_ln(t1p, d, tw[i, "wo"], L.bo, M, d, 1.0, x, L.ln_conv, t0p, tag="out_proj")
            else:
                self._tc(t1p, d, tw[i, "wo"], L.bo, M, d, d, EPI_RESIDUAL, 1.0, x, d, C=x, ldc=d, tag="out_proj")
            if fuse:
                self._tc(t0p, d, tw[i, "pw1"], L.pw1_b, M, 2 * d, d, EPI_BIAS_GLU, C=g, ldc=d, tag="pw1_glu")
            else:
                self._ln_tc(x, L.ln_conv, t0p, tw[i, "pw1"], L.pw1_b, M, 2 * d, EPI_BIAS_GLU, C=g, ldc=d, tag="pw1_glu")
            self._k("dwconv_ln_silu", "masr_dwconv_ln_silu_f32", _p(g), d, T, _p(L.dw), _p(L.dw_b), _p(L.cn[0]),
                    _p(L.cn[1]), _p(L.glu_pad) if self.causal else None, None, _p(t1p[0]), _p(t1p[1]), d, T, _p(tlens), B,
                    d, w.kernel, lpad, T, 1e-5)
            if fuse:
                self._tc_ln(t1p, d, tw[i, "pw2"], L.pw2_b, M, d, 1.0, x, L.ln_ff, t0p, tag="pw2")
            else:
                self._tc(t1p, d, tw[i, "pw2"], L.pw2_b, M, d, d, EPI_RESIDUAL, 1.0, x, d, C=x, ldc=d, tag="pw2")
            if fuse:
                self._tc(t0p, d, tw[i, "ff1"], L.ff[1], M, w.ffn, d, EPI_BIAS_SILU, Cp=hidp, ldc=w.ffn, tag="ffn_w1")
            elif ffn_fused:
                self._ln_split(x, L.ln_ff, t0p, M)
                self._ffn_tc(t0p, tw[i, "ff1"], L.ff[1], tw[i, "ff2"], L.ff[3], M, x)
            else:
                self._ln_tc(x, L.ln_ff, t0p, tw[i, "ff1"], L.ff[1], M, w.ffn, EPI_BIAS_SILU, Cp=hidp, ldc=w.ffn, tag="ffn_w1")
            nxt = w.layers[i + 1].ln_ffm if i + 1 < nl else w.after_norm
            y2 = None if i + 1 < nl else ws["t0"]
            if fuse:
                self._tc_ln(hidp, w.ffn, tw[i, "ff2"], L.ff[3], M, w.ffn, 0.5, x, L.ln_final, t0p, ln2=nxt, y2=y2, tag="ffn_w2")
            else:
                if not ffn_fused:
                    self._tc(hidp, w.ffn, tw[i, "ff2"], L.ff[3], M, d, w.ffn, EPI_RESIDUAL, 0.5, x, d, C=x, ldc=d, tag="ffn_w2")
                self._k("layernorm", "masr_layernorm2_split_f16", _p(x), d, _p(L.ln_final[0]), _p(L.ln_final[1]), _p(x), _p(nxt[0]),
                        _p(nxt[1]), _p(y2), _p(t0p[0]), _p(t0p[1]), d, M, d, 1e-5)
        return ws["t0"][:M], tl, T, ws

    def _ctc_operand(self, ws):
        return ws["t0p"], self.d

    def ctc_logits(self, enc: torch.Tensor, ws) -> torch.Tensor:
        M = enc.shape[0]
        if self.gemm_path == "tc":
            self._tc(ws["t0p"], self.d, self._tcw["ctc"], self.w.ctc_b, M, self.V, self.d, C=ws["logits"], ldc=self.Vpad,
                     tag="ctc_head")
        else:
            self._gemm(enc, self.d, self.w.ctc_w, self.w.ctc_b, ws["logits"], self.Vpad, M, self.V, self.d, tag="ctc_head")
        return ws["logits"]

    def ctc_greedy(self, enc: torch.Tensor, out_lens: Sequence[int], T: int, ws, want_probs: bool = False):
        B = len(out_lens)
        M = B * T
        probs = None
        if self.gemm_path == "tc" and self.fuse_ctc and not want_probs:
            Ap, K = self._ctc_operand(ws)
            need = 3 * ((self.V + 31) // 32) * M * 4
            if ws.get("ctc_part") is None or ws["ctc_part"].numel() < need:
                ws["ctc_part"] = torch.empty(need, device=self.device, dtype=torch.uint8)
            self._k("ctc_head", "masr_ctc_head_argmax_tc_f16x2", _p(Ap[0]), _p(Ap[1]), K, _p(self._tcw["ctc"][0]),
                    _p(self._tcw["ctc"][1]), _p(self.w.ctc_b), M, self.V, K, _p(ws["ctc_part"]), ws["ctc_part"].numel(),
                    _p(ws["ids"]), _p(ws["maxp"]), n=2)
        else:
            logits = self.ctc_logits(enc, ws)
            probs = torch.empty(M, self.V, device=self.device, dtype=torch.float32) if want_probs else None
            self._k("ctc_argmax", "masr_ctc_frame_argmax_f32", _p(logits), self.Vpad, M, self.V, _p(ws["ids"]),
                    _p(ws["maxp"]), _p(probs), self.V)
        self._k("ctc_collapse", "masr_ctc_greedy_collapse", _p(ws["ids"]), _p(ws["maxp"]), T, _p(ws["tlens"]), B, 0,
                _p(ws["tokens"]), ws["tokens"].shape[1], _p(ws["ntok"]), _p(ws["psum"]), _p(ws["pcount"]))
        return probs

    def ctc_beam(self, enc: torch.Tensor, out_lens: Sequence[int], T: int, ws, beam_size: int = 300,
                 cutoff_prob: float = 0.99, cutoff_top_n: int = 40, lm=None, alpha: float = 0.0, beta: float = 0.0):
        B = len(out_lens)
        M = B * T
        dev = self.device
        logits = self.ctc_logits(enc, ws)
        if "cand_id" not in ws or ws["cand_id"].shape[0] < M:
            ws["cand_id"] = torch.empty(M, 40, device=dev, dtype=torch.int32)
            ws["cand_lp"] = torch.empty(M, 40, device=dev, dtype=torch.float32)
            ws["cand_n"] = torch.empty(M, device=dev, dtype=torch.int32)
            pool_n, trie_n = _lib.C.c_int64(0), _lib.C.c_int64(0)
            call("masr_ctc_prefix_beam_workspace", B, T, _lib.C.byref(pool_n), _lib.C.byref(trie_n))
            ws["beam_pool"] = torch.empty(pool_n.value, device=dev, dtype=torch.float32)
            ws["trie_par"] = torch.empty(B * trie_n.value, device=dev, dtype=torch.int32)
            ws["trie_tok"] = torch.empty(B * trie_n.value, device=dev, dtype=torch.int32)
            ws["trie_cap"] = trie_n.value
            ws["beam_tok"] = torch.zeros(B, max(1, T), device=dev, dtype=torch.int32)
            ws["beam_n"] = torch.zeros(B, device=dev, dtype=torch.int32)
            ws["beam_score"] = torch.zeros(B, device=dev, dtype=torch.float32)
        if lm is not None:
            if ws.get("blank_lp") is None or ws["blank_lp"].numel() < M:
                ws["blank_lp"] = torch.empty(M, device=dev, dtype=torch.float32)
            if ws.get("beam_approx") is None or ws["beam_approx"].numel() < ws["beam_score"].numel():
                ws["beam_approx"] = torch.zeros_like(ws["beam_score"])
            self._k("ctc_topk", "masr_ctc_topk_blank_f32", _p(logits), self.Vpad, M, self.V, int(cutoff_top_n), float(cutoff_prob),
                    0, _p(ws["cand_id"]), _p(ws["cand_lp"]), _p(ws["cand_n"]), _p(ws["blank_lp"]))
            self._k("prefix_beam", "masr_ctc_prefix_beam_lm", _p(ws["cand_id"]), _p(ws["cand_lp"]), _p(ws["cand_n"]),
                    _p(ws["blank_lp"]), T, _p(ws["tlens"]), B, int(beam_size), 0, _lib.C.byref(lm.tables(dev)), float(alpha),
                    float(beta), _p(ws["beam_pool"]), _p(ws["trie_par"]), _p(ws["trie_tok"]), ws["trie_cap"], _p(ws["beam_tok"]),
                    ws["beam_tok"].shape[1], _p(ws["beam_n"]), _p(ws["beam_score"]), _p(ws["beam_approx"]))
            self._last_beam = (ws, T, B)
            return ws["beam_tok"], ws["beam_n"], ws["beam_approx"]
        self._k("ctc_topk", "masr_ctc_topk_f32", _p(logits), self.Vpad, M, self.V, int(cutoff_top_n), float(cutoff_prob),
                _p(ws["cand_id"]), _p(ws["cand_lp"]), _p(ws["cand_n"]))
        self._k("prefix_beam", "masr_ctc_prefix_beam", _p(ws["cand_id"]), _p(ws["cand_lp"]), _p(ws["cand_n"]), T, _p(ws["tlens"]),
                B, int(beam_size), 0, _p(ws["beam_pool"]), _p(ws["trie_par"]), _p(ws["trie_tok"]), ws["trie_cap"],
                _p(ws["beam_tok"]), ws["beam_tok"].shape[1], _p(ws["beam_n"]), _p(ws["beam_score"]))
        self._last_beam = (ws, T, B)
        return ws["beam_tok"], ws["beam_n"], ws["beam_score"]

    def last_beam_candidates(self):
        ws, T, B = self._last_beam
        n = ws["cand_n"][:B * T].cpu().numpy().reshape(B, T)
        ids = ws["cand_id"][:B * T].cpu().numpy().reshape(B, T, -1)
        lp = ws["cand_lp"][:B * T].cpu().numpy().reshape(B, T, -1)
        return [[[(int(ids[b, t, k]), np.float32(lp[b, t, k])) for k in range(int(n[b, t]))] for t in range(T)] for b in range(B)]

    def transcribe_beam(self, waves: Sequence[np.ndarray], beam_size: int = 300, cutoff_prob: float = 0.99,
                        cutoff_top_n: int = 40, use_db_normalization: bool = True, target_db: float = -20.0, lm=None,
                        alpha: float = 0.0, beta: float = 0.0, rates: Optional[Sequence[int]] = None):
        feats, frames, status = self.fbank(waves, use_db_normalization, target_db, rates=rates)
        return self.beam_features(feats, frames, beam_size, cutoff_prob, cutoff_top_n, lm, alpha, beta)

    def transcribe_beam_pipelined(self, batches, beam_size: int = 300, cutoff_prob: float = 0.99, cutoff_top_n: int = 40,
                                  use_db_normalization: bool = True, target_db: float = -20.0, lm=None, alpha: float = 0.0,
                                  beta: float = 0.0, with_rates: bool = False):
        dev = self.device
        lm_t = _lib.C.byref(lm.tables(dev)) if lm is not None else None
        main = torch.cuda.current_stream(dev)
        if getattr(self, "_beam_stream", None) is None:
            self._beam_stream = torch.cuda.Stream(device=dev)
            self._beam_slots = [dict(), dict()]
        side = self._beam_stream
        prev = None
        k = 0

        def finish(item):
            slot, B = item
            if B == 0:
                return [], []
            slot["done"].synchronize()
            n = slot["h_n"][:B].numpy()
            tok = slot["h_tok"][:B].numpy()
            sc = slot["h_sc"][:B].numpy()
            self.d2h_bytes += tok.nbytes + n.nbytes + sc.nbytes
            return [tok[b, :n[b]].tolist() for b in range(B)], [float(x) for x in sc]

        for waves in batches:
            waves, rates = waves if with_rates else (waves, None)
            slot = self._beam_slots[k & 1]
            k += 1
            B = len(waves)
            if B == 0:
                item = (slot, 0)
            else:
                if "done" in slot:
                    main.wait_event(slot["done"])
                feats, frames, status = self.fbank(waves, use_db_normalization, target_db, rates=rates)
                enc, tl, T, ws = self.encode(feats, frames)
                M = B * max(1, T)
                if slot.get("M", 0) < M or slot.get("B", 0) < B or slot.get("T", 0) < T:
                    pool_n, trie_n = _lib.C.c_int64(0), _lib.C.c_int64(0)
                    call("masr_ctc_prefix_beam_workspace", B, max(1, T), _lib.C.byref(pool_n), _lib.C.byref(trie_n))
                    i32, f32 = torch.int32, torch.float32
                    slot.update(M=M, B=B, T=T, trie_cap=trie_n.value,
                                cand_id=torch.empty(M, 40, device=dev, dtype=i32), cand_lp=torch.empty(M, 40, device=dev, dtype=f32),
                                cand_n=torch.empty(M, device=dev, dtype=i32), pool=torch.empty(pool_n.value, device=dev, dtype=f32),
                                trie_par=torch.empty(B * trie_n.value, device=dev, dtype=i32),
                                trie_tok=torch.empty(B * trie_n.value, device=dev, dtype=i32),
                                tok=torch.zeros(B, max(1, T), device=dev, dtype=i32), n=torch.zeros(B, device=dev, dtype=i32),
                                sc=torch.zeros(B, device=dev, dtype=f32), tlens=torch.zeros(B, device=dev, dtype=i32),
                                h_tok=torch.zeros(B, max(1, T), dtype=i32, pin_memory=True), h_n=torch.zeros(B, dtype=i32, pin_memory=True),
                                h_sc=torch.zeros(B, dtype=f32, pin_memory=True), ready=torch.cuda.Event(), done=torch.cuda.Event(),
                                blank_lp=torch.empty(M, device=dev, dtype=f32), fused=torch.zeros(B, device=dev, dtype=f32))
                if T == 0:
                    slot["h_n"][:B].zero_()
                    slot["h_sc"][:B].zero_()
                    slot["done"].record(main)
                    item = (slot, B)
                else:
                    logits = self.ctc_logits(enc, ws)
                    if lm_t is None:
                        self._k("ctc_topk", "masr_ctc_topk_f32", _p(logits), self.Vpad, B * T, self.V, int(cutoff_top_n),
                                float(cutoff_prob), _p(slot["cand_id"]), _p(slot["cand_lp"]), _p(slot["cand_n"]))
                    else:
                        self._k("ctc_topk", "masr_ctc_topk_blank_f32", _p(logits), self.Vpad, B * T, self.V, int(cutoff_top_n),
                                float(cutoff_prob), 0, _p(slot["cand_id"]), _p(slot["cand_lp"]), _p(slot["cand_n"]), _p(slot["blank_lp"]))
                    slot["tlens"][:B].copy_(ws["tlens"][:B])
                    slot["ready"].record(main)
                    side.wait_event(slot["ready"])
                    with torch.cuda.stream(side):
                        if lm_t is None:
                            self._k("prefix_beam", "masr_ctc_prefix_beam", _p(slot["cand_id"]), _p(slot["cand_lp"]), _p(slot["cand_n"]), T,
                                    _p(slot["tlens"]), B, int(beam_size), 0, _p(slot["pool"]), _p(slot["trie_par"]), _p(slot["trie_tok"]),
                                    slot["trie_cap"], _p(slot["tok"]), slot["tok"].shape[1], _p(slot["n"]), _p(slot["sc"]))
                        else:
                            self._k("prefix_beam", "masr_ctc_prefix_beam_lm", _p(slot["cand_id"]), _p(slot["cand_lp"]),
                                    _p(slot["cand_n"]), _p(slot["blank_lp"]), T, _p(slot["tlens"]), B, int(beam_size), 0, lm_t,
                                    float(alpha), float(beta), _p(slot["pool"]), _p(slot["trie_par"]), _p(slot["trie_tok"]),
                                    slot["trie_cap"], _p(slot["tok"]), slot["tok"].shape[1], _p(slot["n"]), _p(slot["fused"]),
                                    _p(slot["sc"]))
                        slot["h_tok"][:B, :slot["tok"].shape[1]].copy_(slot["tok"][:B], non_blocking=True)
                        slot["h_n"][:B].copy_(slot["n"][:B], non_blocking=True)
                        slot["h_sc"][:B].copy_(slot["sc"][:B], non_blocking=True)
                        slot["done"].record(side)
                    item = (slot, B)
            if prev is not None:
                yield finish(prev)
            prev = item
        if prev is not None:
            yield finish(prev)

    def beam_features(self, feats, frames, beam_size: int = 300, cutoff_prob: float = 0.99, cutoff_top_n: int = 40, lm=None,
                      alpha: float = 0.0, beta: float = 0.0):
        B = feats.shape[0]
        enc, tl, T, ws = self.encode(feats, frames)
        if T == 0:
            return [[] for _ in range(B)], [0.0] * B
        tok, n, sc = self.ctc_beam(enc, tl, T, ws, beam_size, cutoff_prob, cutoff_top_n, lm, alpha, beta)
        tok, n, sc = tok.cpu().numpy(), n.cpu().numpy(), sc.cpu().numpy()
        self.d2h_bytes += tok.nbytes + n.nbytes + sc.nbytes
        return [tok[b, :n[b]].tolist() for b in range(B)], [float(s) for s in sc]

    def transcribe(self, waves: Sequence[np.ndarray], use_db_normalization: bool = True, target_db: float = -20.0,
                   return_frames: bool = False, rates: Optional[Sequence[int]] = None) -> GreedyResult:
        if self.use_graphs and self.prof is None and len(waves) > 0:
            return self._transcribe_graph(waves, use_db_normalization, target_db, return_frames, rates)
        feats, frames, status = self.fbank(waves, use_db_normalization, target_db, rates=rates)
        return self.transcribe_features(feats, frames, status, return_frames)

    def final_len(self, t: int) -> int:
        return t

    GRAPH_FRAME_QUANTUM = 32
    PIPE_DEPTH = 3
    STAGE_THREADS = 4

    def _graph_for(self, B: int, Fpad: int, use_db: bool, target_db: float, slot: int = 0):
        key = (B, Fpad, use_db, float(target_db), slot)
        g = self._graphs.get(key)
        if g is not None:
            return g
        dev = self.device
        cap_samples = (Fpad - 1) * FRAME_SHIFT + FRAME_LEN + FRAME_SHIFT - 1
        g = {
            "wave": torch.zeros(B * cap_samples + 8, device=dev, dtype=torch.float32),
            "offs": torch.zeros(B + 1, device=dev, dtype=torch.int64),
            "tlens": torch.zeros(B, device=dev, dtype=torch.int32),
            "cap_samples": cap_samples,
        }
        lengths = [cap_samples] * B
        g["offs"].copy_(torch.arange(B + 1, dtype=torch.int64) * cap_samples)
        frames = [Fpad] * B

        def body():
            ws0 = self._workspace(B, Fpad)
            feats, _, status = self.fbank(None, use_db, target_db, wave_dev=g["wave"], offsets_dev=g["offs"],
                                          lengths=lengths, force_fmax=Fpad, status_out=ws0["status"])
            enc, tl, T, ws = self.encode(feats, frames, tlens_dev=g["tlens"])
            self.ctc_greedy(enc, tl, T, ws)
            if self.graph_tail_hook is not None:
                self.graph_tail_hook(ws)
            return ws, status, T

        g["tlens"].fill_(subsampled_len(Fpad))
        side = torch.cuda.Stream(device=dev)
        side.wait_stream(torch.cuda.current_stream(dev))
        with torch.cuda.stream(side):
            body()
        torch.cuda.current_stream(dev).wait_stream(side)
        torch.cuda.synchronize(dev)
        n0 = self.launches
        graph = torch.cuda.CUDAGraph()
        with torch.cuda.graph(graph, capture_error_mode="thread_local"):
            g["ws"], g["status"], g["T"] = body()
        g["launches"] = self.launches - n0
        self.launches = n0
        g["graph"] = graph
        if len(self._graphs) >= 16:
            self._graphs.pop(next(iter(self._graphs)))
        self._graphs[key] = g
        return g

    def transcribe_pipelined(self, batches, use_db_normalization: bool = True, target_db: float = -20.0, device_hook=None,
                             with_rates: bool = False):
        dev = self.device
        comp = torch.cuda.current_stream(dev)
        if getattr(self, "_copy_stream", None) is None:
# ... 510 lines not shown
```

Before: 41810.

## Fuse LayerNorm into FFN and row-block GEMMs, add dwconv+pw2+LN kernel

New measurement: 43370 (median of 6 runs). +3.8%, better.

```diff
diff --git a/include/masr_b200.h b/include/masr_b200.h
--- a/include/masr_b200.h
+++ b/include/masr_b200.h
@@ -66,6 +66,22 @@
 int masr_ffn_tc_f16x2(const void* Ah, const void* Al, int64_t lda, const void* W1h, const void* W1l, const float* b1,
                       const void* W2h, const void* W2l, const float* b2, float* x, int64_t ldx, int M, int D, int F,
                       float alpha, void* stream);
+
+int masr_ffn_tc_ln_f16x2(const void* Ah, const void* Al, int64_t lda, const void* W1h, const void* W1l, const float* b1,
+                         const void* W2h, const void* W2l, const float* b2, float* x, int64_t ldx, int M, int D, int F,
+                         float alpha, const float* gamma1, const float* beta1, const float* gamma2, const float* beta2,
+                         float* Y2, void* Yh, void* Yl, int64_t ldy, float eps, void* stream);
+
+int masr_rowblock_tc_ln_f16x2(const void* Ah, const void* Al, int64_t lda, const void* Wh, const void* Wl, const float* bias,
+                              float* x, int64_t ldx, float alpha, const float* gamma1, const float* beta1,
+                              const float* gamma2, const float* beta2, float* Y2, void* Yh, void* Yl, int64_t ldy,
+                              int M, int N, int K, float eps, void* stream);
+
+int masr_rowblock_dwconv_tc_ln_f16x2(const float* g, int T, const int* in_lens, const float* dw_w, const float* dw_b,
+                                     const float* cn_gamma, const float* cn_beta, const float* pad_vec, int kernel_size, int lpad,
+                                     float cn_eps, const void* Wh, const void* Wl, const float* bias, float* x, int64_t ldx,
+                                     float alpha, const float* gamma1, const float* beta1, const float* gamma2, const float* beta2,
+                                     float* Y2, void* Yh, void* Yl, int64_t ldy, int M, int N, int K, float eps, void* stream);
 
 int masr_gemm_tc_residual_ln_f16x2(const void* Ah, const void* Al, int64_t lda, const void* Wh, const void* Wl,
                                    const float* bias, const float* residual, int64_t ldr, float alpha, float* X,
diff --git a/masr_b200/_lib.py b/masr_b200/_lib.py
--- a/masr_b200/_lib.py
+++ b/masr_b200/_lib.py
@@ -36,6 +36,12 @@
     "masr_gemm_f32": [_vp, _i64, _vp, _vp, _vp, _i64, _vp, _i64, _i, _i, _i, _i, _f, _vp],
     "masr_gemm_tc_f16x2": [_vp, _vp, _i64, _vp, _vp, _vp, _vp, _i64, _vp, _vp, _vp, _i64, _i, _i, _i, _i, _f, _vp],
     "masr_ffn_tc_f16x2": [_vp, _vp, _i64, _vp, _vp, _vp, _vp, _vp, _vp, _vp, _i64, _i, _i, _i, _f, _vp],
+    "masr_ffn_tc_ln_f16x2": [_vp, _vp, _i64, _vp, _vp, _vp, _vp, _vp, _vp, _vp, _i64, _i, _i, _i, _f, _vp, _vp, _vp, _vp, _vp, _vp,
+                             _vp, _i64, _f, _vp],
+    "masr_rowblock_dwconv_tc_ln_f16x2": [_vp, _i, _vp, _vp, _vp, _vp, _vp, _vp, _i, _i, _f, _vp, _vp, _vp, _vp, _i64, _f, _vp, _vp,
+                                         _vp, _vp, _vp, _vp, _vp, _i64, _i, _i, _i, _f, _vp],
+    "masr_rowblock_tc_ln_f16x2": [_vp, _vp, _i64, _vp, _vp, _vp, _vp, _i64, _f, _vp, _vp, _vp, _vp, _vp, _vp, _vp, _i64, _i, _i, _i,
+                                  _f, _vp],
     "masr_gemm_tc_residual_ln_f16x2": [_vp, _vp, _i64, _vp, _vp, _vp, _vp, _i64, _f, _vp, _vp, _vp, _vp, _vp, _vp, _vp, _vp, _i64,
                                        _i, _i, _i, _f, _vp],
     "masr_gemm_tc_residual_postln_f16x2": [_vp, _vp, _i64, _vp, _vp, _vp, _vp, _i64, _f, _vp, _vp, _vp, _vp, _vp, _vp, _vp, _i64,
diff --git a/masr_b200/csrc/ffn_tc.cu b/masr_b200/csrc/ffn_tc.cu
--- a/masr_b200/csrc/ffn_tc.cu
+++ b/masr_b200/csrc/ffn_tc.cu
@@ -37,6 +37,7 @@
     int64_t ldx;
     int M, F;
     float alpha;
+    RowLnParams ln;
 };
 
 __device__ __forceinline__ void wgmma_m64n64k16_ss(float (&d)[32], uint64_t da, uint64_t db, uint32_t scale_d) {
@@ -57,6 +58,7 @@
 
 __device__ __forceinline__ void bar_consumers() { asm volatile("bar.sync 1, 256;" ::: "memory"); }
 
+template <bool LN>
 __global__ void __launch_bounds__(F_THREADS, 1) ffn_tc_kernel(const __grid_constant__ FfnMaps maps, FfnParams p) {
     extern __shared__ uint8_t smem_raw[];
     uint8_t* smem = reinterpret_cast<uint8_t*>((reinterpret_cast<uintptr_t>(smem_raw) + 1023) & ~uintptr_t(1023));
@@ -120,9 +122,8 @@
     } else {
         setmaxnreg_inc<F_CONSUMER_REGS>();
         const int wg = warp >> 2, wi = warp & 3, q = lane & 3;
-        const int tid = threadIdx.x & 127;
         const uint32_t h_base = smem_u32(hbuf);
-        const uint32_t sum_base = smem_u32(sum) + wg * (F_SUM_BYTES / 2) + tid * 8;
+        const uint32_t sum_base = smem_u32(sum) + wg * (F_SUM_BYTES / 2) + (threadIdx.x & 127) * 8;
         const uint32_t is_lane0 = lane == 0;
         auto release = [&](uint32_t s) {
             asm volatile("{\n\t.reg .pred p;\n\tsetp.ne.u32 p, %1, 0;\n\t@p mbarrier.arrive.shared::cta.b64 _, [%0];\n\t}"
@@ -185,6 +186,7 @@
             }
         };
         const int r_lo = 16 * wi + (lane >> 2);
+        auto sum_addr = [&](int i, int hh) { return sum_base + (i * 2 + hh) * 1024; };
         auto store_hidden = [&](int j) {
             float2 bb[8];
             const float* b = p.b1 + j * FHC + 64 * wg + 2 * q;
@@ -237,7 +239,7 @@
 #pragma unroll
                         for (int hh = 0; hh < 2; ++hh) {
                             float x0 = acc2[4 * i + 2 * hh], x1 = acc2[4 * i + 2 * hh + 1];
-                            const uint32_t a = sum_base + (i * 2 + hh) * 1024;
+                            const uint32_t a = sum_addr(i, hh);
                             if (j > 1) {
                                 float s0, s1;
                                 asm volatile("ld.shared.v2.f32 {%0, %1}, [%2];" : "=f"(s0), "=f"(s1) : "r"(a) : "memory");
@@ -261,7 +263,7 @@
                     float x0 = acc2[4 * i + 2 * hh], x1 = acc2[4 * i + 2 * hh + 1];
                     if (nch > 2) {
                         float s0, s1;
-                        asm volatile("ld.shared.v2.f32 {%0, %1}, [%2];" : "=f"(s0), "=f"(s1) : "r"(sum_base + (i * 2 + hh) * 1024) : "memory");
+                        asm volatile("ld.shared.v2.f32 {%0, %1}, [%2];" : "=f"(s0), "=f"(s1) : "r"(sum_addr(i, hh)) : "memory");
                         x0 = s0 + x0; x1 = s1 + x1;
                     }
                     x0 = fmaf(cor2[4 * i + 2 * hh], kLoInv, x0);
@@ -273,30 +275,25 @@
                         const float2 r = *xp;
                         x0 = r.x + p.alpha * x0;
                         x1 = r.y + p.alpha * x1;
-                        *xp = make_float2(x0, x1);
+                        if (!LN) *xp = make_float2(x0, x1);
                     }
-                }
+                    if (LN) asm volatile("st.shared.v2.f32 [%0], {%1, %2};" ::"r"(sum_addr(i, hh)), "f"(x0), "f"(x1) : "memory");
+                }
+            }
+            if (LN) {
+                bar_consumers();
+                const uint32_t sum0 = smem_u32(sum);
+                row_ln_epilogue<1>([&](int r, int k) {
+                    return sum0 + k * (F_SUM_BYTES / 2) + (((r >> 4) * 32 + (r & 7) * 4 + 2 * (lane & 1)) * 8) +
+                           ((lane >> 1) * 2 + ((r >> 3) & 1)) * 1024;
+                }, m0, p.M, warp, lane, p.x, p.ldx, p.ln);
             }
         }
     }
     __syncthreads();
 }
 
-int ffn_map(CUtensorMap* map, const void* ptr, int64_t rows, int64_t K, int64_t ld, int box_rows) {
-    EncodeTiledFn fn = get_encode_fn();
-    if (!fn) { set_last_error("cuTensorMapEncodeTiled entry point unavailable"); return MASR_ERR_INTERNAL; }
-    cuuint64_t dims[2] = {(cuuint64_t)K, (cuuint64_t)rows};
-    cuuint64_t strides[1] = {(cuuint64_t)ld * 2};
-    cuuint32_t box[2] = {(cuuint32_t)FBK, (cuuint32_t)box_rows};
-    cuuint32_t estr[2] = {1, 1};
-    CUresult r = fn(map, CU_TENSOR_MAP_DATA_TYPE_FLOAT16, 2, const_cast<void*>(ptr), dims, strides, box, estr,
-                    CU_TENSOR_MAP_INTERLEAVE_NONE, CU_TENSOR_MAP_SWIZZLE_64B, CU_TENSOR_MAP_L2_PROMOTION_L2_128B,
-                    CU_TENSOR_MAP_FLOAT_OOB_FILL_NONE);
-    if (r != CUDA_SUCCESS) { set_last_error("cuTensorMapEncodeTiled failed (%d) rows=%lld K=%lld ld=%lld", (int)r, (long long)rows, (long long)K, (long long)ld); return MASR_ERR_INTERNAL; }
-    return MASR_OK;
-}
-
-bool g_ffn_attr_set[64] = {false};
+bool g_ffn_attr_set[2][64] = {{false}};
 
 }
 
@@ -304,10 +301,9 @@
 
 using namespace masr;
 
-extern "C" int masr_ffn_tc_f16x2(const void* Ah, const void* Al, int64_t lda, const void* W1h, const void* W1l, const float* b1,
-                                 const void* W2h, const void* W2l, const float* b2, float* x, int64_t ldx, int M, int D, int F,
-                                 float alpha, void* stream) {
-    if (M == 0) return MASR_OK;
+static int launch_ffn(const void* Ah, const void* Al, int64_t lda, const void* W1h, const void* W1l, const float* b1,
+                      const void* W2h, const void* W2l, const float* b2, float* x, int64_t ldx, int M, int D, int F,
+                      float alpha, const RowLnParams& ln, void* stream) {
     MASR_REQUIRE(Ah && Al && W1h && W1l && b1 && W2h && W2l && b2 && x, "masr_ffn_tc_f16x2: null pointer");
     MASR_REQUIRE(M > 0, "masr_ffn_tc_f16x2: M=%d", M);
     MASR_REQUIRE(D == FD, "masr_ffn_tc_f16x2: D=%d unsupported (this build: %d)", D, FD);
@@ -321,24 +317,50 @@
     FfnMaps maps;
     memset(&maps, 0, sizeof(maps));
     int rc;
-    if ((rc = ffn_map(&maps.xh, Ah, M, D, lda, FM))) return rc;
-    if ((rc = ffn_map(&maps.xl, Al, M, D, lda, FM))) return rc;
-    if ((rc = ffn_map(&maps.w1h, W1h, F, D, D, FHC))) return rc;
-    if ((rc = ffn_map(&maps.w1l, W1l, F, D, D, FHC))) return rc;
-    if ((rc = ffn_map(&maps.w2h, W2h, D, F, F, FD))) return rc;
-    if ((rc = ffn_map(&maps.w2l, W2l, D, F, F, FD))) return rc;
+    if ((rc = tma_map_k32(&maps.xh, Ah, M, D, lda, FM))) return rc;
+    if ((rc = tma_map_k32(&maps.xl, Al, M, D, lda, FM))) return rc;
+    if ((rc = tma_map_k32(&maps.w1h, W1h, F, D, D, FHC))) return rc;
+    if ((rc = tma_map_k32(&maps.w1l, W1l, F, D, D, FHC))) return rc;
+    if ((rc = tma_map_k32(&maps.w2h, W2h, D, F, F, FD))) return rc;
+    if ((rc = tma_map_k32(&maps.w2l, W2l, D, F, F, FD))) return rc;
     int dev = 0;
     cudaGetDevice(&dev);
     if (dev < 0 || dev >= 64) dev = 0;
-    if (!g_ffn_attr_set[dev]) {
-        cudaError_t e = cudaFuncSetAttribute(ffn_tc_kernel, cudaFuncAttributeMaxDynamicSharedMemorySize, (int)kFfnSmem);
+    const bool lnk = ln.g1 != nullptr;
+    if (!g_ffn_attr_set[lnk][dev]) {
+        cudaError_t e = cudaFuncSetAttribute(lnk ? ffn_tc_kernel<true> : ffn_tc_kernel<false>,
+                                             cudaFuncAttributeMaxDynamicSharedMemorySize, (int)kFfnSmem);
         if (e != cudaSuccess) { set_last_error("ffn_tc smem attr: %s", cudaGetErrorString(e)); return (int)e; }
-        g_ffn_attr_set[dev] = true;
+        g_ffn_attr_set[lnk][dev] = true;
     }
     int sms = 0;
     if (cudaDeviceGetAttribute(&sms, cudaDevAttrMultiProcessorCount, dev) != cudaSuccess || sms <= 0) sms = 132;
     const int nrb = (M + FM - 1) / FM;
-    FfnParams p{b1, b2, x, ldx, M, F, alpha};
-    launch_pdl(ffn_tc_kernel, dim3(nrb < sms ? nrb : sms), dim3(F_THREADS), kFfnSmem, (cudaStream_t)stream, maps, p);
+    FfnParams p{b1, b2, x, ldx, M, F, alpha, ln};
+    const dim3 grid(nrb < sms ? nrb : sms);
+    if (lnk) {
+        launch_pdl(ffn_tc_kernel<true>, grid, dim3(F_THREADS), kFfnSmem, (cudaStream_t)stream, maps, p);
+        return check_launch("ffn_tc_kernel<ln>");
+    }
+    launch_pdl(ffn_tc_kernel<false>, grid, dim3(F_THREADS), kFfnSmem, (cudaStream_t)stream, maps, p);
     return check_launch("ffn_tc_kernel");
 }
+
+extern "C" int masr_ffn_tc_f16x2(const void* Ah, const void* Al, int64_t lda, const void* W1h, const void* W1l, const float* b1,
+                                 const void* W2h, const void* W2l, const float* b2, float* x, int64_t ldx, int M, int D, int F,
+                                 float alpha, void* stream) {
+    if (M == 0) return MASR_OK;
+    RowLnParams ln;
+    memset(&ln, 0, sizeof(ln));
+    return launch_ffn(Ah, Al, lda, W1h, W1l, b1, W2h, W2l, b2, x, ldx, M, D, F, alpha, ln, stream);
+}
+
+extern "C" int masr_ffn_tc_ln_f16x2(const void* Ah, const void* Al, int64_t lda, const void* W1h, const void* W1l, const float* b1,
+                                    const void* W2h, const void* W2l, const float* b2, float* x, int64_t ldx, int M, int D, int F,
+                                    float alpha, const float* gamma1, const float* beta1, const float* gamma2, const float* beta2,
+                                    float* Y2, void* Yh, void* Yl, int64_t ldy, float eps, void* stream) {
+    if (M == 0) return MASR_OK;
+    RowLnParams ln;
+    if (int rc = check_row_ln("masr_ffn_tc_ln_f16x2", x, ldx, gamma1, beta1, gamma2, beta2, Y2, Yh, Yl, ldy, eps, &ln)) return rc;
+    return launch_ffn(Ah, Al, lda, W1h, W1l, b1, W2h, W2l, b2, x, ldx, M, D, F, alpha, ln, stream);
+}
diff --git a/masr_b200/csrc/rowblock_tc.cu b/masr_b200/csrc/rowblock_tc.cu
--- /dev/null
+++ b/masr_b200/csrc/rowblock_tc.cu
@@ -0,0 +1,345 @@
+#include <cuda.h>
+#include <cuda_fp16.h>
+#include <string.h>
+
+#include "tc_common.cuh"
+
+namespace masr {
+
+namespace {
+
+constexpr int RM = 64;
+constexpr int RD = 256;
+constexpr int RBK = 32;
+constexpr int R_STAGES = 4;
+constexpr int R_A_BYTES = RM * RBK * 2;
+constexpr int R_W_BYTES = RD * RBK * 2;
+constexpr int R_STAGE_BYTES = 2 * R_A_BYTES + 2 * R_W_BYTES;
+constexpr int R_THREADS = 384;
+constexpr int R_PRODUCER_REGS = 40, R_CONSUMER_REGS = 232;
+constexpr int R_DW_K = 15;
+constexpr int R_TAP_BYTES = R_DW_K * RD * 4;
+constexpr int R_DW_TW = 2;
+template <bool CONV> constexpr int kRowStage = CONV ? 2 * R_W_BYTES : R_STAGE_BYTES;
+template <bool CONV> constexpr int kRowWOff = CONV ? 0 : 2 * R_A_BYTES;
+template <bool CONV>
+constexpr size_t kRowSmem = R_STAGES * kRowStage<CONV> + kRowStageBytes + (CONV ? R_TAP_BYTES : 0) + 1024 + 256;
+static_assert(kRowSmem<false> <= 232448 && kRowSmem<true> <= 232448, "rowblock_tc shared memory exceeds the 227 KB per-CTA limit of sm_90");
+static_assert(R_PRODUCER_REGS * 128 + R_CONSUMER_REGS * 256 <= 65536, "register file of the SM");
+
+struct RowMaps {
+    CUtensorMap ah, al;
+    CUtensorMap wh, wl;
+};
+
+struct RowParams {
+    const float* bias;
+    float* x;
+    int64_t ldx;
+    int M;
+    float alpha;
+    RowLnParams ln;
+    const float* g;
+    const float* dw_w;
+    const float* dw_b;
+    const float* cn_g;
+    const float* cn_b;
+    const float* pad_vec;
+    const int* in_lens;
+    int T, lpad;
+    float cn_eps;
+};
+
+__device__ __forceinline__ void store_a4(uint32_t a_base, int r, int c, const float (&o)[4]) {
+    __half hh[4], ll[4];
+#pragma unroll
+    for (int e = 0; e < 4; ++e) {
+        hh[e] = __float2half_rn(o[e]);
+        ll[e] = __float2half_rn((o[e] - __half2float(hh[e])) * 2048.0f);
+    }
+    const uint32_t a = a_base + (c >> 5) * 8192 + r * 64 + ((((c & 31) >> 3) ^ ((r >> 1) & 3)) << 4) + (c & 7) * 2;
+    const uint2 h = *reinterpret_cast<const uint2*>(hh), l = *reinterpret_cast<const uint2*>(ll);
+    asm volatile("st.shared.v2.b32 [%0], {%1, %2};" ::"r"(a), "r"(h.x), "r"(h.y) : "memory");
+    asm volatile("st.shared.v2.b32 [%0], {%1, %2};" ::"r"(a + 4096), "r"(l.x), "r"(l.y) : "memory");
+}
+
+template <int TW>
+__device__ __forceinline__ void dw_rows(const RowParams& p, const float* s_w, uint32_t a_base, int r0, int m, int lane) {
+    constexpr int C = 256, ROWS = TW - 1 + R_DW_K;
+    const int b = m / p.T, t0 = m - b * p.T;
+    const int in_len = __ldg(p.in_lens + b);
+    const int c0 = lane * 4, c1 = 128 + lane * 4;
+    const float4 bs0 = ldg_f4(p.dw_b + c0), bs1 = ldg_f4(p.dw_b + c1);
+    float4 pv0 = make_float4(0.f, 0.f, 0.f, 0.f), pv1 = pv0;
+    if (p.pad_vec) { pv0 = ldg_f4(p.pad_vec + c0); pv1 = ldg_f4(p.pad_vec + c1); }
+    float4 a0[TW], a1[TW];
+#pragma unroll
+    for (int j = 0; j < TW; ++j) { a0[j] = bs0; a1[j] = bs1; }
+    const float* gb = p.g + (int64_t)b * p.T * C;
+#pragma unroll
+    for (int i = 0; i < ROWS; ++i) {
+        const int tau = t0 - p.lpad + i;
+        float4 v0, v1;
+        if (tau < 0) { v0 = pv0; v1 = pv1; }
+        else if (tau >= in_len) { v0 = make_float4(0.f, 0.f, 0.f, 0.f); v1 = v0; }
+        else { v0 = ldg_f4(gb + (int64_t)tau * C + c0); v1 = ldg_f4(gb + (int64_t)tau * C + c1); }
+#pragma unroll
+        for (int j = 0; j < TW; ++j) {
+            const int k = i - j;
+            if (k >= 0 && k < R_DW_K) {
+                const float4 w0 = *reinterpret_cast<const float4*>(s_w + k * C + c0);
+                const float4 w1 = *reinterpret_cast<const float4*>(s_w + k * C + c1);
+                a0[j].x = fmaf(w0.x, v0.x, a0[j].x); a0[j].y = fmaf(w0.y, v0.y, a0[j].y);
+                a0[j].z = fmaf(w0.z, v0.z, a0[j].z); a0[j].w = fmaf(w0.w, v0.w, a0[j].w);
+                a1[j].x = fmaf(w1.x, v1.x, a1[j].x); a1[j].y = fmaf(w1.y, v1.y, a1[j].y);
+                a1[j].z = fmaf(w1.z, v1.z, a1[j].z); a1[j].w = fmaf(w1.w, v1.w, a1[j].w);
+            }
+        }
+    }
+    const float4 gg0 = ldg_f4(p.cn_g + c0), gg1 = ldg_f4(p.cn_g + c1), bb0 = ldg_f4(p.cn_b + c0), bb1 = ldg_f4(p.cn_b + c1);
+#pragma unroll
+    for (int j = 0; j < TW; ++j) {
+        const float mean = warp_sum(((a0[j].x + a0[j].y) + (a0[j].z + a0[j].w)) + ((a1[j].x + a1[j].y) + (a1[j].z + a1[j].w))) * (1.0f / C);
+        const float d0 = a0[j].x - mean, d1 = a0[j].y - mean, d2 = a0[j].z - mean, d3 = a0[j].w - mean;
+        const float d4 = a1[j].x - mean, d5 = a1[j].y - mean, d6 = a1[j].z - mean, d7 = a1[j].w - mean;
+        const float q = ((d0 * d0 + d1 * d1) + (d2 * d2 + d3 * d3)) + ((d4 * d4 + d5 * d5) + (d6 * d6 + d7 * d7));
+        const float rstd = rsqrtf(warp_sum(q) * (1.0f / C) + p.cn_eps);
+        const float o0[4] = {fast_silu((a0[j].x - mean) * rstd * gg0.x + bb0.x), fast_silu((a0[j].y - mean) * rstd * gg0.y + bb0.y),
+                             fast_silu((a0[j].z - mean) * rstd * gg0.z + bb0.z), fast_silu((a0[j].w - mean) * rstd * gg0.w + bb0.w)};
+        const float o1[4] = {fast_silu((a1[j].x - mean) * rstd * gg1.x + bb1.x), fast_silu((a1[j].y - mean) * rstd * gg1.y + bb1.y),
+                             fast_silu((a1[j].z - mean) * rstd * gg1.z + bb1.z), fast_silu((a1[j].w - mean) * rstd * gg1.w + bb1.w)};
+        store_a4(a_base, r0 + j, c0, o0);
+        store_a4(a_base, r0 + j, c1, o1);
+    }
+}
+
+__device__ __forceinline__ void bar_consumers() { asm volatile("bar.sync 1, 256;" ::: "memory"); }
+
+template <bool CONV>
+__global__ void __launch_bounds__(R_THREADS, 1) rowblock_tc_ln_kernel(const __grid_constant__ RowMaps maps, RowParams p) {
+    extern __shared__ uint8_t smem_raw[];
+    uint8_t* smem = reinterpret_cast<uint8_t*>((reinterpret_cast<uintptr_t>(smem_raw) + 1023) & ~uintptr_t(1023));
+    constexpr int SB = kRowStage<CONV>;
+    uint8_t* stage = smem + R_STAGES * SB;
+    float* s_w = reinterpret_cast<float*>(stage + kRowStageBytes);
+    uint64_t* full_bar = reinterpret_cast<uint64_t*>(stage + kRowStageBytes + (CONV ? R_TAP_BYTES : 0));
+    uint64_t* empty_bar = full_bar + R_STAGES;
+
+    const int warp = threadIdx.x >> 5, lane = threadIdx.x & 31;
+    const int nrb = (p.M + RM - 1) / RM;
+    if (CONV) {
+        for (int idx = threadIdx.x; idx < R_DW_K * RD; idx += R_THREADS) {
+            const int k = idx / RD, c = idx - k * RD;
+            s_w[idx] = __ldg(p.dw_w + c * R_DW_K + k);
+        }
+    }
+
+    if (warp == 8 && lane == 0) {
+        if (!CONV) { tma_prefetch_desc(&maps.ah); tma_prefetch_desc(&maps.al); }
+        tma_prefetch_desc(&maps.wh); tma_prefetch_desc(&maps.wl);
+        for (int s = 0; s < R_STAGES; ++s) { mbar_init(&full_bar[s], 1); mbar_init(&empty_bar[s], 8); }
+        asm volatile("fence.mbarrier_init.release.cluster;" ::: "memory");
+    }
+    __syncthreads();
+    pdl_wait();
+    pdl_launch_dependents();
+
+    if (warp >= 8) {
+        setmaxnreg_dec<R_PRODUCER_REGS>();
+        if (warp == 8 && elect_one_sync()) {
+            uint32_t kg = 0;
+            for (int rb = blockIdx.x; rb < nrb; rb += gridDim.x) {
+#pragma unroll 1
+                for (int kb = 0; kb < RD / RBK; ++kb, ++kg) {
+                    const uint32_t s = kg % R_STAGES;
+                    mbar_wait(&empty_bar[s], ((kg / R_STAGES) & 1) ^ 1);
+                    mbar_expect_tx(&full_bar[s], SB);
+                    uint8_t* st = smem + s * SB;
+                    if (!CONV) {
+                        tma_load_2d(&maps.ah, &full_bar[s], st, kb * RBK, rb * RM);
+                        tma_load_2d(&maps.al, &full_bar[s], st + R_A_BYTES, kb * RBK, rb * RM);
+                    }
+                    tma_load_2d(&maps.wh, &full_bar[s], st + kRowWOff<CONV>, kb * RBK, 0);
+                    tma_load_2d(&maps.wl, &full_bar[s], st + kRowWOff<CONV> + R_W_BYTES, kb * RBK, 0);
+                }
+            }
+        }
+        __syncwarp();
+    } else {
+        setmaxnreg_inc<R_CONSUMER_REGS>();
+        const int wg = warp >> 2, wi = warp & 3, q = lane & 3;
+        const uint32_t stage_base = smem_u32(stage);
+        const uint32_t is_lane0 = lane == 0;
+        auto release = [&](uint32_t s) {
+            asm volatile("{\n\t.reg .pred p;\n\tsetp.ne.u32 p, %1, 0;\n\t@p mbarrier.arrive.shared::cta.b64 _, [%0];\n\t}"
+                         ::"r"(smem_u32(&empty_bar[s])), "r"(is_lane0) : "memory");
+        };
+        const int r_lo = 16 * wi + (lane >> 2);
+        float acc[64], cor[64];
+        uint32_t kg = 0;
+        for (int rb = blockIdx.x; rb < nrb; rb += gridDim.x) {
+            const int m0 = rb * RM;
+            if (CONV) {
+                bar_consumers();
+#pragma unroll 1
+                for (int gi = 0; gi < 8 / R_DW_TW; ++gi) {
+                    const int r0 = warp * 8 + gi * R_DW_TW, m = m0 + r0;
+                    if (m + R_DW_TW - 1 < p.M && m / p.T == (m + R_DW_TW - 1) / p.T) {
+                        dw_rows<R_DW_TW>(p, s_w, stage_base, r0, m, lane);
+                    } else {
+#pragma unroll 1
+                        for (int j = 0; j < R_DW_TW; ++j) {
+                            if (m + j < p.M) {
+                                dw_rows<1>(p, s_w, stage_base, r0 + j, m + j, lane);
+                            } else {
+                                const float z[4] = {0.f, 0.f, 0.f, 0.f};
+                                store_a4(stage_base, r0 + j, lane * 4, z);
+                                store_a4(stage_base, r0 + j, 128 + lane * 4, z);
+                            }
+                        }
+                    }
+                }
+                asm volatile("fence.proxy.async.shared::cta;" ::: "memory");
+                bar_consumers();
+            }
+            int pend = -1;
+#pragma unroll 1
+            for (int kb = 0; kb < RD / RBK; ++kb, ++kg) {
+                const uint32_t s = kg % R_STAGES;
+                mbar_wait(&full_bar[s], (kg / R_STAGES) & 1);
+                const uint32_t sa = smem_u32(smem + s * SB);
+                const uint32_t sA = CONV ? stage_base + kb * 8192 : sa;
+                const uint64_t dAh = gmma_desc_sw64(sA), dAl = gmma_desc_sw64(sA + (CONV ? 4096 : R_A_BYTES));
+                const uint32_t sw = sa + kRowWOff<CONV> + wg * (R_W_BYTES / 2);
+                const uint64_t dWh = gmma_desc_sw64(sw), dWl = gmma_desc_sw64(sw + R_W_BYTES);
+                reg_fence(acc); reg_fence(cor);
+                wgmma_fence();
+#pragma unroll
+                for (int ks = 0; ks < RBK / 16; ++ks) {
+                    const uint64_t adv = (uint64_t)(ks * 2);
+                    const uint32_t acc_on = (kb | ks) ? 1u : 0u;
+                    wgmma_m64n128k16_ss(acc, dAh + adv, dWh + adv, acc_on);
+                    wgmma_m64n128k16_ss(cor, dAh + adv, dWl + adv, acc_on);
+                    wgmma_m64n128k16_ss(cor, dAl + adv, dWh + adv, 1u);
+                }
+                wgmma_commit();
+                wgmma_wait<1>();
+                reg_fence(acc); reg_fence(cor);
+                if (pend >= 0) release((uint32_t)pend);
+                pend = (int)s;
+            }
+            wgmma_wait<0>();
+            reg_fence(acc); reg_fence(cor);
+            release((uint32_t)pend);
+            bar_consumers();
+            const float* bias = p.bias + 128 * wg + 2 * q;
+#pragma unroll
+            for (int i = 0; i < 16; ++i) {
+                const float2 bv = __ldg(reinterpret_cast<const float2*>(bias + 8 * i));
+#pragma unroll
+                for (int hh = 0; hh < 2; ++hh) {
+                    float x0 = fmaf(cor[4 * i + 2 * hh], kLoInv, acc[4 * i + 2 * hh]);
+                    float x1 = fmaf(cor[4 * i + 2 * hh + 1], kLoInv, acc[4 * i + 2 * hh + 1]);
+                    x0 += bv.x; x1 += bv.y;
+                    const int r = r_lo + 8 * hh, c = 128 * wg + 8 * i + 2 * q;
+                    if (m0 + r < p.M) {
+                        const float2 rv = *reinterpret_cast<const float2*>(p.x + (int64_t)(m0 + r) * p.ldx + c);
+                        x0 = rv.x + p.alpha * x0;
+                        x1 = rv.y + p.alpha * x1;
+                    }
+                    asm volatile("st.shared.v2.f32 [%0], {%1, %2};" ::"r"(stage_base + row_stage_off(r, c)), "f"(x0), "f"(x1) : "memory");
+                }
+            }
+            bar_consumers();
+            row_ln_epilogue<4>([&](int r, int k) { return stage_base + row_stage_off(r, (k * 32 + lane) * 4); }, m0, p.M, warp,
+                              lane, p.x, p.ldx, p.ln);
+        }
+    }
+    __syncthreads();
+}
+
+bool g_row_attr_set[2][64] = {{false}};
+
+template <bool CONV>
+int launch_rowblock(const RowMaps& maps, const RowParams& p, cudaStream_t stream) {
+    int dev = 0;
+    cudaGetDevice(&dev);
+    if (dev < 0 || dev >= 64) dev = 0;
+    if (!g_row_attr_set[CONV][dev]) {
+        cudaError_t e = cudaFuncSetAttribute(rowblock_tc_ln_kernel<CONV>, cudaFuncAttributeMaxDynamicSharedMemorySize, (int)kRowSmem<CONV>);
+        if (e != cudaSuccess) { set_last_error("rowblock_tc smem attr: %s", cudaGetErrorString(e)); return (int)e; }
+        g_row_attr_set[CONV][dev] = true;
+    }
+    int sms = 0;
+    if (cudaDeviceGetAttribute(&sms, cudaDevAttrMultiProcessorCount, dev) != cudaSuccess || sms <= 0) sms = 132;
+    const int nrb = (p.M + RM - 1) / RM;
+    launch_pdl(rowblock_tc_ln_kernel<CONV>, dim3(nrb < sms ? nrb : sms), dim3(R_THREADS), kRowSmem<CONV>, stream, maps, p);
+    return check_launch(CONV ? "rowblock_tc_ln_kernel<conv>" : "rowblock_tc_ln_kernel");
+}
+
+}
+
+}
+
+using namespace masr;
+
+extern "C" int masr_rowblock_tc_ln_f16x2(const void* Ah, const void* Al, int64_t lda, const void* Wh, const void* Wl, const float* bias,
+                                         float* x, int64_t ldx, float alpha, const float* gamma1, const float* beta1,
+                                         const float* gamma2, const float* beta2, float* Y2, void* Yh, void* Yl, int64_t ldy,
+                                         int M, int N, int K, float eps, void* stream) {
+    if (M == 0) return MASR_OK;
+    MASR_REQUIRE(Ah && Al && Wh && Wl && bias && x, "masr_rowblock_tc_ln_f16x2: null pointer");
+    MASR_REQUIRE(M > 0, "masr_rowblock_tc_ln_f16x2: M=%d", M);
+    MASR_REQUIRE(N == RD && K == RD, "masr_rowblock_tc_ln_f16x2: N=%d K=%d unsupported (this build: %d)", N, K, RD);
+    MASR_REQUIRE(lda >= K && lda % 8 == 0, "masr_rowblock_tc_ln_f16x2: lda=%lld must be >= %d and a multiple of 8", (long long)lda, K);
+    MASR_REQUIRE(ldx >= N, "masr_rowblock_tc_ln_f16x2: ldx=%lld must be >= %d", (long long)ldx, N);
+    MASR_REQUIRE(ldy >= N, "masr_rowblock_tc_ln_f16x2: ldy=%lld must be >= %d", (long long)ldy, N);
+    MASR_REQUIRE(((reinterpret_cast<uintptr_t>(Ah) | reinterpret_cast<uintptr_t>(Al) | reinterpret_cast<uintptr_t>(Wh) |
+                   reinterpret_cast<uintptr_t>(Wl)) & 15) == 0 && (reinterpret_cast<uintptr_t>(bias) & 7) == 0,
+                 "masr_rowblock_tc_ln_f16x2: misaligned pointer");
+    RowParams p;
+    memset(&p, 0, sizeof(p));
+    p.bias = bias; p.x = x; p.ldx = ldx; p.M = M; p.alpha = alpha;
+    if (int rc = check_row_ln("masr_rowblock_tc_ln_f16x2", x, ldx, gamma1, beta1, gamma2, beta2, Y2, Yh, Yl, ldy, eps, &p.ln)) return rc;
+    RowMaps maps;
+    memset(&maps, 0, sizeof(maps));
+    int rc;
+    if ((rc = tma_map_k32(&maps.ah, Ah, M, K, lda, RM))) return rc;
+    if ((rc = tma_map_k32(&maps.al, Al, M, K, lda, RM))) return rc;
+    if ((rc = tma_map_k32(&maps.wh, Wh, N, K, K, RD))) return rc;
+    if ((rc = tma_map_k32(&maps.wl, Wl, N, K, K, RD))) return rc;
+    return launch_rowblock<false>(maps, p, (cudaStream_t)stream);
+}
+
+extern "C" int masr_rowblock_dwconv_tc_ln_f16x2(const float* g, int T, const int* in_lens, const float* dw_w, const float* dw_b,
+                                                const float* cn_gamma, const float* cn_beta, const float* pad_vec, int kernel_size,
+                                                int lpad, float cn_eps, const void* Wh, const void* Wl, const float* bias, float* x,
+                                                int64_t ldx, float alpha, const float* gamma1, const float* beta1, const float* gamma2,
+                                                const float* beta2, float* Y2, void* Yh, void* Yl, int64_t ldy, int M, int N, int K,
+                                                float eps, void* stream) {
+    if (M == 0) return MASR_OK;
+    MASR_REQUIRE(g && in_lens && dw_w && dw_b && cn_gamma && cn_beta && Wh && Wl && bias && x,
+                 "masr_rowblock_dwconv_tc_ln_f16x2: null pointer");
+    MASR_REQUIRE(M > 0 && T > 0 && M % T == 0, "masr_rowblock_dwconv_tc_ln_f16x2: M=%d must be a positive multiple of T=%d", M, T);
+    MASR_REQUIRE(N == RD && K == RD, "masr_rowblock_dwconv_tc_ln_f16x2: N=%d K=%d unsupported (this build: %d)", N, K, RD);
+    MASR_REQUIRE(kernel_size == R_DW_K && lpad >= 0 && lpad < R_DW_K,
+                 "masr_rowblock_dwconv_tc_ln_f16x2: kernel_size=%d lpad=%d unsupported (kernel %d, 0 <= lpad < kernel)", kernel_size, lpad, R_DW_K);
+    MASR_REQUIRE(ldx >= N && ldy >= N, "masr_rowblock_dwconv_tc_ln_f16x2: ldx=%lld ldy=%lld must be >= %d", (long long)ldx, (long long)ldy, N);
+    MASR_REQUIRE(((reinterpret_cast<uintptr_t>(g) | reinterpret_cast<uintptr_t>(dw_b) | reinterpret_cast<uintptr_t>(cn_gamma) |
+                   reinterpret_cast<uintptr_t>(cn_beta) | reinterpret_cast<uintptr_t>(pad_vec) | reinterpret_cast<uintptr_t>(Wh) |
+                   reinterpret_cast<uintptr_t>(Wl)) & 15) == 0 && (reinterpret_cast<uintptr_t>(bias) & 7) == 0,
+                 "masr_rowblock_dwconv_tc_ln_f16x2: misaligned pointer");
+    RowParams p;
+    memset(&p, 0, sizeof(p));
+    p.bias = bias; p.x = x; p.ldx = ldx; p.M = M; p.alpha = alpha;
+    p.g = g; p.dw_w = dw_w; p.dw_b = dw_b; p.cn_g = cn_gamma; p.cn_b = cn_beta; p.pad_vec = pad_vec; p.in_lens = in_lens;
+    p.T = T; p.lpad = lpad; p.cn_eps = cn_eps;
+    if (int rc = check_row_ln("masr_rowblock_dwconv_tc_ln_f16x2", x, ldx, gamma1, beta1, gamma2, beta2, Y2, Yh, Yl, ldy, eps, &p.ln))
+        return rc;
+    RowMaps maps;
+    memset(&maps, 0, sizeof(maps));
+    int rc;
+    if ((rc = tma_map_k32(&maps.wh, Wh, N, K, K, RD))) return rc;
+    if ((rc = tma_map_k32(&maps.wl, Wl, N, K, K, RD))) return rc;
+    return launch_rowblock<true>(maps, p, (cudaStream_t)stream);
+}
diff --git a/masr_b200/csrc/tc_common.cuh b/masr_b200/csrc/tc_common.cuh
--- a/masr_b200/csrc/tc_common.cuh
+++ b/masr_b200/csrc/tc_common.cuh
@@ -134,6 +134,115 @@
     return v;
 }
 
+__device__ __forceinline__ void ln_row256(const float4 (&v)[2], const float* __restrict__ gamma, const float* __restrict__ beta,
+                                          float eps, int lane, float4 (&o)[2]) {
+    float s = 0.f;
+#pragma unroll
+    for (int i = 0; i < 2; ++i) s += (v[i].x + v[i].y) + (v[i].z + v[i].w);
+    const float mean = warp_sum(s) * (1.0f / 256);
+    float q = 0.f;
+#pragma unroll
+    for (int i = 0; i < 2; ++i) {
+        float a = v[i].x - mean, b = v[i].y - mean, c = v[i].z - mean, d = v[i].w - mean;
+        q += (a * a + b * b) + (c * c + d * d);
+    }
+    const float rstd = rsqrtf(warp_sum(q) * (1.0f / 256) + eps);
+#pragma unroll
+    for (int i = 0; i < 2; ++i) {
+        const int c = (i * 32 + lane) * 4;
+        float4 g = ldg_f4(gamma + c), b = ldg_f4(beta + c);
+        o[i].x = (v[i].x - mean) * rstd * g.x + b.x;
+        o[i].y = (v[i].y - mean) * rstd * g.y + b.y;
+        o[i].z = (v[i].z - mean) * rstd * g.z + b.z;
+        o[i].w = (v[i].w - mean) * rstd * g.w + b.w;
+    }
+}
+
+__device__ __forceinline__ void store_pair_row256(const float4 (&o)[2], int lane, __half* __restrict__ yh, __half* __restrict__ yl) {
+#pragma unroll
+    for (int i = 0; i < 2; ++i) {
+        const int c = (i * 32 + lane) * 4;
+        __half hh[4], ll[4];
+        const float ov[4] = {o[i].x, o[i].y, o[i].z, o[i].w};
+#pragma unroll
+        for (int j = 0; j < 4; ++j) {
+            hh[j] = __float2half_rn(ov[j]);
+            ll[j] = __float2half_rn((ov[j] - __half2float(hh[j])) * 2048.0f);
+        }
+        *reinterpret_cast<uint2*>(yh + c) = *reinterpret_cast<const uint2*>(hh);
+        *reinterpret_cast<uint2*>(yl + c) = *reinterpret_cast<const uint2*>(ll);
+    }
+}
+
+constexpr int kRowStageBytes = 64 * 256 * 4;
+__device__ __forceinline__ uint32_t row_stage_off(int r, int c) {
+    return (uint32_t)(r * 1024 + ((((c >> 2) ^ (r & 7))) << 4) + (c & 3) * 4);
+}
+
+struct RowLnParams {
+    const float* g1;
+    const float* b1;
+    const float* g2;
+    const float* b2;
+    float* y2;
+    __half* yh;
+    __half* yl;
+    int64_t ldy;
+    float eps;
+};
+
+template <int RIF, typename Addr>
+__device__ __forceinline__ void row_ln_epilogue(Addr addr, int m0, int M, int warp, int lane, float* x, int64_t ldx,
+                                                const RowLnParams& a) {
+#pragma unroll 1
+    for (int r4 = 0; r4 < 8; r4 += RIF) {
+        float4 v[RIF][2];
+#pragma unroll
+        for (int k = 0; k < RIF; ++k)
+#pragma unroll
+            for (int i = 0; i < 2; ++i) {
+                const int r = warp * 8 + r4 + k;
+                const uint4 u = lds128(addr(r, i));
+                v[k][i] = make_float4(__uint_as_float(u.x), __uint_as_float(u.y), __uint_as_float(u.z), __uint_as_float(u.w));
+            }
+#pragma unroll
+        for (int k = 0; k < RIF; ++k) {
+            const int row = m0 + warp * 8 + r4 + k;
+            if (row >= M) break;
+            float4 o[2];
+            ln_row256(v[k], a.g1, a.b1, a.eps, lane, o);
+            float* xr = x + (int64_t)row * ldx;
+            if (a.g2) {
+#pragma unroll
+                for (int i = 0; i < 2; ++i) *reinterpret_cast<float4*>(xr + (i * 32 + lane) * 4) = o[i];
+                v[k][0] = o[0]; v[k][1] = o[1];
+                ln_row256(v[k], a.g2, a.b2, a.eps, lane, o);
+            } else {
+#pragma unroll
+                for (int i = 0; i < 2; ++i) *reinterpret_cast<float4*>(xr + (i * 32 + lane) * 4) = v[k][i];
+            }
+            if (a.y2) {
+#pragma unroll
+                for (int i = 0; i < 2; ++i) *reinterpret_cast<float4*>(a.y2 + (int64_t)row * a.ldy + (i * 32 + lane) * 4) = o[i];
+            }
+            store_pair_row256(o, lane, a.yh + (int64_t)row * a.ldy, a.yl + (int64_t)row * a.ldy);
+        }
+    }
+}
+
+inline int check_row_ln(const char* fn, const float* x, int64_t ldx, const float* g1, const float* b1, const float* g2,
+                        const float* b2, float* y2, void* yh, void* yl, int64_t ldy, float eps, RowLnParams* out) {
+    MASR_REQUIRE(g1 && b1 && yh && yl, "%s: null pointer", fn);
+    MASR_REQUIRE((g2 == nullptr) == (b2 == nullptr), "%s: gamma2/beta2 must come as a pair", fn);
+    MASR_REQUIRE(ldx % 4 == 0 && ldy % 4 == 0, "%s: ldx=%lld and ldy=%lld must be multiples of 4", fn, (long long)ldx, (long long)ldy);
+    MASR_REQUIRE(((reinterpret_cast<uintptr_t>(x) | reinterpret_cast<uintptr_t>(g1) | reinterpret_cast<uintptr_t>(b1) |
+                   reinterpret_cast<uintptr_t>(g2) | reinterpret_cast<uintptr_t>(b2) | reinterpret_cast<uintptr_t>(y2)) & 15) == 0 &&
+                 ((reinterpret_cast<uintptr_t>(yh) | reinterpret_cast<uintptr_t>(yl)) & 7) == 0,
+                 "%s: misaligned LayerNorm operand", fn);
+    *out = RowLnParams{g1, b1, g2, b2, y2, static_cast<__half*>(yh), static_cast<__half*>(yl), ldy, eps};
+    return MASR_OK;
+}
+
 typedef CUresult (*EncodeTiledFn)(CUtensorMap*, CUtensorMapDataType, cuuint32_t, void*, const cuuint64_t*, const cuuint64_t*,
                                   const cuuint32_t*, const cuuint32_t*, CUtensorMapInterleave, CUtensorMapSwizzle,
                                   CUtensorMapL2promotion, CUtensorMapFloatOOBfill);
@@ -151,4 +260,18 @@
     return fn;
 }
 
-}
+inline int tma_map_k32(CUtensorMap* map, const void* ptr, int64_t rows, int64_t K, int64_t ld, int box_rows) {
+    EncodeTiledFn fn = get_encode_fn();
+    if (!fn) { set_last_error("cuTensorMapEncodeTiled entry point unavailable"); return MASR_ERR_INTERNAL; }
+    cuuint64_t dims[2] = {(cuuint64_t)K, (cuuint64_t)rows};
+    cuuint64_t strides[1] = {(cuuint64_t)ld * 2};
+    cuuint32_t box[2] = {32, (cuuint32_t)box_rows};
+    cuuint32_t estr[2] = {1, 1};
+    CUresult r = fn(map, CU_TENSOR_MAP_DATA_TYPE_FLOAT16, 2, const_cast<void*>(ptr), dims, strides, box, estr,
+                    CU_TENSOR_MAP_INTERLEAVE_NONE, CU_TENSOR_MAP_SWIZZLE_64B, CU_TENSOR_MAP_L2_PROMOTION_L2_128B,
+                    CU_TENSOR_MAP_FLOAT_OOB_FILL_NONE);
+    if (r != CUDA_SUCCESS) { set_last_error("cuTensorMapEncodeTiled failed (%d) rows=%lld K=%lld ld=%lld", (int)r, (long long)rows, (long long)K, (long long)ld); return MASR_ERR_INTERNAL; }
+    return MASR_OK;
+}
+
+}
diff --git a/masr_b200/csrc/tc_gemm.cu b/masr_b200/csrc/tc_gemm.cu
--- a/masr_b200/csrc/tc_gemm.cu
+++ b/masr_b200/csrc/tc_gemm.cu
@@ -50,36 +50,9 @@
 
 __device__ __forceinline__ void ln_row256_split(const float4 (&v)[2], const float* __restrict__ gamma, const float* __restrict__ beta,
                                                 float eps, int lane, __half* __restrict__ yh, __half* __restrict__ yl) {
-    float s = 0.f;
-#pragma unroll
-    for (int i = 0; i < 2; ++i) s += (v[i].x + v[i].y) + (v[i].z + v[i].w);
-    const float mean = warp_sum(s) * (1.0f / 256);
-    float q = 0.f;
-#pragma unroll
-    for (int i = 0; i < 2; ++i) {
-        float a = v[i].x - mean, b = v[i].y - mean, c = v[i].z - mean, d = v[i].w - mean;
-        q += (a * a + b * b) + (c * c + d * d);
-    }
-    const float rstd = rsqrtf(warp_sum(q) * (1.0f / 256) + eps);
-#pragma unroll
-    for (int i = 0; i < 2; ++i) {
-        const int c = (i * 32 + lane) * 4;
-        float4 g = ldg_f4(gamma + c), b = ldg_f4(beta + c);
-        float4 o;
-        o.x = (v[i].x - mean) * rstd * g.x + b.x;
-        o.y = (v[i].y - mean) * rstd * g.y + b.y;
-        o.z = (v[i].z - mean) * rstd * g.z + b.z;
-        o.w = (v[i].w - mean) * rstd * g.w + b.w;
-        __half hh[4], ll[4];
-        const float ov[4] = {o.x, o.y, o.z, o.w};
-#pragma unroll
-        for (int j = 0; j < 4; ++j) {
-            hh[j] = __float2half_rn(ov[j]);
-            ll[j] = __float2half_rn((ov[j] - __half2float(hh[j])) * 2048.0f);
-        }
-        *reinterpret_cast<uint2*>(yh + c) = *reinterpret_cast<const uint2*>(hh);
-        *reinterpret_cast<uint2*>(yl + c) = *reinterpret_cast<const uint2*>(ll);
-    }
+    float4 o[2];
+    ln_row256(v, gamma, beta, eps, lane, o);
+    store_pair_row256(o, lane, yh, yl);
 }
 
 constexpr int EPI_RESIDUAL_LN = 6, EPI_RESIDUAL_LN2 = 7, EPI_CTC_PARTIAL = 8, EPI_RESIDUAL_POSTLN = 9;
diff --git a/masr_b200/engine.py b/masr_b200/engine.py
--- a/masr_b200/engine.py
+++ b/masr_b200/engine.py
@@ -54,6 +54,7 @@
         self.attn_tc5 = os.environ.get("MASR_ATTN", "tc5") != "mma"
         self.fuse = os.environ.get("MASR_FUSE_LN", "0") == "1"
         self.lnpre = os.environ.get("MASR_FUSE_LNPRE", "0") == "1"
+        self.rowfuse = os.environ.get("MASR_ROWFUSE", "1") != "0"
         self.use_graphs = bool(use_graphs)
         self._graphs = {}
         if not torch.cuda.is_available():
@@ -155,6 +156,17 @@
         d = self.d
         self._k("ffn_fused", "masr_ffn_tc_f16x2", _p(A[0]), _p(A[1]), d, _p(W1[0]), _p(W1[1]), _p(b1), _p(W2[0]), _p(W2[1]),
                 _p(b2), _p(x), d, M, d, self.w.ffn, alpha)
+
+    def _ffn_tc_ln(self, A, W1, b1, W2, b2, M, x, ln1, yp, ln2=None, y2=None, alpha=0.5):
+        d = self.d
+        self._k("ffn_fused", "masr_ffn_tc_ln_f16x2", _p(A[0]), _p(A[1]), d, _p(W1[0]), _p(W1[1]), _p(b1), _p(W2[0]), _p(W2[1]),
+                _p(b2), _p(x), d, M, d, self.w.ffn, alpha, _p(ln1[0]), _p(ln1[1]), None if ln2 is None else _p(ln2[0]),
+                None if ln2 is None else _p(ln2[1]), _p(y2), _p(yp[0]), _p(yp[1]), d, 1e-5)
+
+    def _row_ln(self, A, W, bias, M, x, ln, yp, tag):
+        d = self.d
+        self._k(tag, "masr_rowblock_tc_ln_f16x2", _p(A[0]), _p(A[1]), d, _p(W[0]), _p(W[1]), _p(bias), _p(x), d, 1.0,
+                _p(ln[0]), _p(ln[1]), None, None, None, _p(yp[0]), _p(yp[1]), d, M, d, d, 1e-5)
 
     def _hidp(self, ws):
         if "hidp" not in ws:
@@ -469,6 +481,27 @@
                  tag="embed_linear")
         lpad = (w.kernel - 1) if self.causal else (w.kernel - 1) // 2
         nl = len(w.layers)
+        if ffn_fused and self.rowfuse:
+            self._ln_split(x, w.layers[0].ln_ffm, t0p, M)
+            for i, L in enumerate(w.layers):
+                self._ffn_tc_ln(t0p, tw[i, "ffm1"], L.ffm[1], tw[i, "ffm2"], L.ffm[3], M, x, L.ln_mha, t0p)
+                self._tc(t0p, d, tw[i, "qkv"], L.bqkv, M, 3 * d, d, C=qkv, Cp=ws["qkvp"], ldc=3 * d, tag="qkv_proj")
+                self._attention_tc(L, qkv, ws["qkvp"], t1p, T, tlens, B)
+                self._row_ln(t1p, tw[i, "wo"], L.bo, M, x, L.ln_conv, t0p, tag="out_proj")
+                self._tc(t0p, d, tw[i, "pw1"], L.pw1_b, M, 2 * d, d, EPI_BIAS_GLU, C=g, ldc=d, tag="pw1_glu")
+                pad = _p(L.glu_pad) if self.causal else None
+                if w.kernel == 15:
+                    self._k("pw2", "masr_rowblock_dwconv_tc_ln_f16x2", _p(g), T, _p(tlens), _p(L.dw), _p(L.dw_b), _p(L.cn[0]),
+                            _p(L.cn[1]), pad, w.kernel, lpad, 1e-5, _p(tw[i, "pw2"][0]), _p(tw[i, "pw2"][1]), _p(L.pw2_b), _p(x),
+                            d, 1.0, _p(L.ln_ff[0]), _p(L.ln_ff[1]), None, None, None, _p(t0p[0]), _p(t0p[1]), d, M, d, d, 1e-5)
+                else:
+                    self._k("dwconv_ln_silu", "masr_dwconv_ln_silu_f32", _p(g), d, T, _p(L.dw), _p(L.dw_b), _p(L.cn[0]),
+                            _p(L.cn[1]), pad, None, _p(t1p[0]), _p(t1p[1]), d, T, _p(tlens), B, d, w.kernel, lpad, T, 1e-5)
+                    self._row_ln(t1p, tw[i, "pw2"], L.pw2_b, M, x, L.ln_ff, t0p, tag="pw2")
+                last = i + 1 == nl
+                self._ffn_tc_ln(t0p, tw[i, "ff1"], L.ff[1], tw[i, "ff2"], L.ff[3], M, x, L.ln_final, t0p,
+                                ln2=w.after_norm if last else w.layers[i + 1].ln_ffm, y2=ws["t0"] if last else None)
+            return ws["t0"][:M], tl, T, ws
         for i, L in enumerate(w.layers):
             fuse = self.fuse and d == 256
             if ffn_fused:
```
